# Duankaiwen/LSNet

Hardware: AMD Instinct MI355X
Metric: img/s train LSNet R-50-FPN 1333x800 bs2/GPU (higher is better)
Workload: dtype f32 (fp32-equivalent: 6 bf16 MFMA terms per product on exact 3-way operand splits, fp32 accumulate); 1 GPU; LSNet R50-FPN bbox (conv_module_type=dcn), 2 img/GPU 3x800x1344 (1333x800 padded to /32), 7 gt/img, fwd+bwd+gradient arena (the reducer's buckets, no collective on one rank)+clip35+SGD; global_batch=2, parallelism=dp1, world_size=1, memory_format=channels_last, launch=eager

## Files before the change

include/lsnet_hip.h:

```cpp
#ifndef LSNET_HIP_H_
#define LSNET_HIP_H_

#include <stdint.h>

#ifdef __cplusplus
extern "C" {
#endif

typedef struct ihipStream_t *lsn_stream_t;

typedef enum {
    LSN_OK = 0,
    LSN_ERR_INVALID = -1,
    LSN_ERR_UNSUPPORTED = -2,
    LSN_ERR_RUNTIME = -3
} lsn_status;

typedef enum { LSN_NCHW = 0, LSN_NHWC = 1 } lsn_layout;

typedef struct { int64_t b, c, h, w; } lsn_strides4;

typedef struct {
    int B, C, H, W;
    int Co, Ho, Wo;
    int kh, kw, stride, pad, dil;
    int groups, deformable_groups;
    float scale_h, scale_w;
    int mask_is_logit;
    void *workspace;
    void *gather_workspace;
    int64_t gather_workspace_bytes;
    int accumulate_param_grads;
    int out_pitch;
    int weights_prepared;
} lsn_dcn_shape;

typedef struct {
    const float *input;
    const float *offset;
    const float *mask;
    float *output;
    const float *grad_output;
    float *grad_input;
    float *grad_offset;
    float *grad_mask;
    lsn_strides4 off_st, mask_st;
    int B, H, W, Ho, Wo;
    float scale_h, scale_w;
} lsn_dcn_level;

const char *lsn_last_error(void);
int lsn_version(void);

enum { LSN_MATH_FP32 = 0, LSN_MATH_BF16X3 = 1, LSN_MATH_BF16X6 = 2, LSN_MATH_BF16 = 3 };
int lsn_set_math_mode(int mode);
int lsn_get_math_mode(void);


int lsn_dcn_forward(const lsn_dcn_shape *shape, int n_levels, const lsn_dcn_level *levels,
                    const float *weight, const float *bias, lsn_layout layout, lsn_stream_t stream);

int lsn_dcn_backward(const lsn_dcn_shape *shape, int n_levels, const lsn_dcn_level *levels,
                     const float *weight, float *grad_weight, float *grad_bias, lsn_layout layout,
                     lsn_stream_t stream);

int64_t lsn_dcn_backward_workspace_bytes(const lsn_dcn_shape *shape, int n_levels, const lsn_dcn_level *levels);
int lsn_dcn_pitched_ok(const lsn_dcn_shape *shape, int n_levels, const lsn_dcn_level *levels, int backward);
int lsn_dcn_prepared_ok(const lsn_dcn_shape *shape, int n_levels, const lsn_dcn_level *levels, int backward);
int lsn_dcn_anchor_lists(const lsn_dcn_shape *shape, int n_levels, const lsn_dcn_level *levels, lsn_layout layout,
                         int *sample_anchor, int *list_start, int *list_sample, int64_t *counts, lsn_stream_t stream);


int lsn_deform_conv_forward(const float *input, const float *weight, const float *offset, float *output,
                            int B, int C, int H, int W, int Co, int kW, int kH, int dW, int dH, int padW,
                            int padH, int dilW, int dilH, int group, int deformable_group,
                            int im2col_step, lsn_stream_t stream);
int lsn_deform_conv_backward_input(const float *input, const float *offset, const float *grad_output,
                                   float *grad_input, float *grad_offset, const float *weight, int B,
                                   int C, int H, int W, int Co, int kW, int kH, int dW, int dH, int padW,
                                   int padH, int dilW, int dilH, int group, int deformable_group,
                                   int im2col_step, lsn_stream_t stream);
int lsn_deform_conv_backward_parameters(const float *input, const float *offset, const float *grad_output,
                                        float *grad_weight, int B, int C, int H, int W, int Co, int kW,
                                        int kH, int dW, int dH, int padW, int padH, int dilW, int dilH,
                                        int group, int deformable_group, float scale, int im2col_step,
                                        lsn_stream_t stream);
int lsn_modulated_deform_conv_forward(const float *input, const float *weight, const float *bias,
                                      const float *offset, const float *mask, float *output, int B, int C,
                                      int H, int W, int Co, int kernel_h, int kernel_w, int stride_h,
                                      int stride_w, int pad_h, int pad_w, int dilation_h, int dilation_w,
                                      int group, int deformable_group, int with_bias, lsn_stream_t stream);
int lsn_modulated_deform_conv_backward(const float *input, const float *weight, const float *bias,
                                       const float *offset, const float *mask, float *grad_input,
                                       float *grad_weight, float *grad_bias, float *grad_offset,
                                       float *grad_mask, const float *grad_output, int B, int C, int H,
                                       int W, int Co, int kernel_h, int kernel_w, int stride_h,
                                       int stride_w, int pad_h, int pad_w, int dilation_h, int dilation_w,
                                       int group, int deformable_group, int with_bias,
                                       lsn_stream_t stream);
int lsn_pyramid_deform_conv_forward(const float *input, const float *weight, const float *offset,
                                    float *output, int B, int C, int H, int W, int Co, int Ho, int Wo,
                                    int kW, int kH, int dW, int dH, int padW, int padH, int dilW, int dilH,
                                    float scaleW, float scaleH, int group, int deformable_group,
                                    int im2col_step, lsn_stream_t stream);
int lsn_pyramid_deform_conv_backward_input(const float *input, const float *offset,
                                           const float *grad_output, float *grad_input,
                                           float *grad_offset, const float *weight, int B, int C, int H,
                                           int W, int Co, int Ho, int Wo, int kW, int kH, int dW, int dH,
                                           int padW, int padH, int dilW, int dilH, float scaleW,
                                           float scaleH, int group, int deformable_group,
                                           int im2col_step, lsn_stream_t stream);
int lsn_pyramid_deform_conv_backward_parameters(const float *input, const float *offset,
                                                const float *grad_output, float *grad_weight, int B,
                                                int C, int H, int W, int Co, int Ho, int Wo, int kW,
                                                int kH, int dW, int dH, int padW, int padH, int dilW,
                                                int dilH, float scaleW, float scaleH, int group,
                                                int deformable_group, float scale, int im2col_step,
                                                lsn_stream_t stream);

int lsn_sigmoid_focal_loss_forward(const float *logits, const int64_t *targets, float *losses, int N,
                                   int C, float gamma, float alpha, lsn_stream_t stream);
int lsn_sigmoid_focal_loss_backward(const float *logits, const int64_t *targets, const float *d_losses,
                                    float *d_logits, int N, int C, float gamma, float alpha,
                                    lsn_stream_t stream);
int lsn_sigmoid_focal_loss_sum(const float *logits, const int64_t *targets, const float *weight,
                               float *loss_sum, int N, int C, float gamma, float alpha,
                               lsn_stream_t stream);
int lsn_sigmoid_focal_loss_backward_weighted(const float *logits, const int64_t *targets,
                                             const float *weight, const float *scale, float *d_logits,
                                             int N, int C, float gamma, float alpha, lsn_stream_t stream);

int lsn_sigmoid_focal_loss_level_sums(const float *logits, const int64_t *targets, const float *weight, float *loss_sums,
                                      int B, int N_all, int C, int L, const int *level_starts, float gamma, float alpha,
                                      lsn_stream_t stream);
int lsn_sigmoid_focal_loss_backward_levels(const float *logits, const int64_t *targets, const float *weight, const float *scales,
                                           float *d_logits, int B, int N_all, int C, int L, const int *level_starts,
                                           float gamma, float alpha, lsn_stream_t stream);
int lsn_level_sums(const float *rows, float *sums, int B, int N_all, int L, const int *level_starts, lsn_stream_t stream);
int lsn_level_expand(const float *g, float *out_rows, int B, int N_all, int L, const int *level_starts, lsn_stream_t stream);

typedef struct {
    float *param, *grad, *momentum_buf;
    int64_t numel, first_chunk;
    int group;
} lsn_sgd_tensor;
typedef struct {
    float lr, momentum, weight_decay;
} lsn_sgd_group;
int64_t lsn_clip_sgd_workspace_bytes(void);
int lsn_clip_sgd_step(int n_tensors, const lsn_sgd_tensor *tensors_dev, int64_t total_chunks, int n_groups,
                      const lsn_sgd_group *groups, float max_norm, void *workspace, float *stats, lsn_stream_t stream);

typedef struct {
// ... 286 lines not shown
```

lsnet_amd/_lib.py:

```python
import ctypes
import os

_HERE = os.path.dirname(os.path.abspath(__file__))
SO_PATH = os.environ.get('LSNET_HIP_SO') or os.path.join(_HERE, 'csrc', 'liblsnet_hip.so')


class Strides4(ctypes.Structure):
    c_name = 'lsn_strides4'
    _fields_ = [('b', ctypes.c_int64), ('c', ctypes.c_int64), ('h', ctypes.c_int64), ('w', ctypes.c_int64)]


class DcnShape(ctypes.Structure):
    c_name = 'lsn_dcn_shape'
    _fields_ = [('B', ctypes.c_int), ('C', ctypes.c_int), ('H', ctypes.c_int), ('W', ctypes.c_int),
                ('Co', ctypes.c_int), ('Ho', ctypes.c_int), ('Wo', ctypes.c_int),
                ('kh', ctypes.c_int), ('kw', ctypes.c_int), ('stride', ctypes.c_int), ('pad', ctypes.c_int),
                ('dil', ctypes.c_int), ('groups', ctypes.c_int), ('deformable_groups', ctypes.c_int),
                ('scale_h', ctypes.c_float), ('scale_w', ctypes.c_float), ('mask_is_logit', ctypes.c_int),
                ('workspace', ctypes.c_void_p), ('gather_workspace', ctypes.c_void_p),
                ('gather_workspace_bytes', ctypes.c_int64), ('accumulate_param_grads', ctypes.c_int),
                ('out_pitch', ctypes.c_int), ('weights_prepared', ctypes.c_int)]


class DcnLevel(ctypes.Structure):
    c_name = 'lsn_dcn_level'
    _fields_ = [('input', ctypes.c_void_p), ('offset', ctypes.c_void_p), ('mask', ctypes.c_void_p),
                ('output', ctypes.c_void_p), ('grad_output', ctypes.c_void_p), ('grad_input', ctypes.c_void_p),
                ('grad_offset', ctypes.c_void_p), ('grad_mask', ctypes.c_void_p),
                ('off_st', Strides4), ('mask_st', Strides4),
                ('B', ctypes.c_int), ('H', ctypes.c_int), ('W', ctypes.c_int), ('Ho', ctypes.c_int),
                ('Wo', ctypes.c_int), ('scale_h', ctypes.c_float), ('scale_w', ctypes.c_float)]


class OffsetChainLevel(ctypes.Structure):
    c_name = 'lsn_offset_chain_level'
    _fields_ = [('off', ctypes.c_void_p), ('out', ctypes.c_void_p * 3), ('gout', ctypes.c_void_p * 6), ('goff', ctypes.c_void_p),
                ('images', ctypes.c_int64), ('per_image', ctypes.c_int64), ('off_image_pitch', ctypes.c_int64),
                ('mh', ctypes.c_float * 3), ('mw', ctypes.c_float * 3)]


class WgradBnJob(ctypes.Structure):
    c_name = 'lsn_wgrad_bn_job'
    _fields_ = [('x', ctypes.c_void_p), ('g', ctypes.c_void_p), ('w', ctypes.c_void_p), ('bn_gamma', ctypes.c_void_p),
                ('bn_mean', ctypes.c_void_p), ('bn_var', ctypes.c_void_p), ('bn_eps', ctypes.c_float),
                ('grad_w', ctypes.c_void_p), ('grad_gamma', ctypes.c_void_p), ('grad_beta', ctypes.c_void_p)]


class SgdTensor(ctypes.Structure):
    c_name = 'lsn_sgd_tensor'
    _fields_ = [('param', ctypes.c_void_p), ('grad', ctypes.c_void_p), ('momentum_buf', ctypes.c_void_p),
                ('numel', ctypes.c_int64), ('first_chunk', ctypes.c_int64), ('group', ctypes.c_int)]


class SgdGroup(ctypes.Structure):
    c_name = 'lsn_sgd_group'
    _fields_ = [('lr', ctypes.c_float), ('momentum', ctypes.c_float), ('weight_decay', ctypes.c_float)]


class ConvLevel(ctypes.Structure):
    c_name = 'lsn_conv_level'
    _fields_ = [('x', ctypes.c_void_p), ('out', ctypes.c_void_p), ('grad_out', ctypes.c_void_p),
                ('B', ctypes.c_int), ('H', ctypes.c_int), ('W', ctypes.c_int), ('residual', ctypes.c_void_p),
                ('gate', ctypes.c_void_p)]


class ConvWprep(ctypes.Structure):
    c_name = 'lsn_conv_wprep'
    _fields_ = [('kind', ctypes.c_int), ('w', ctypes.c_void_p), ('prepared', ctypes.c_void_p), ('C', ctypes.c_int),
                ('Co', ctypes.c_int), ('kh', ctypes.c_int), ('kw', ctypes.c_int), ('stride', ctypes.c_int),
                ('pad', ctypes.c_int), ('dil', ctypes.c_int),
                ('bn_gamma', ctypes.c_void_p), ('bn_var', ctypes.c_void_p), ('bn_beta', ctypes.c_void_p),
                ('bn_mean', ctypes.c_void_p), ('shift_out', ctypes.c_void_p), ('bn_eps', ctypes.c_float)]


class GnLevel(ctypes.Structure):
    c_name = 'lsn_gn_level'
    _fields_ = [('x', ctypes.c_void_p), ('y', ctypes.c_void_p), ('dy', ctypes.c_void_p), ('dx', ctypes.c_void_p),
                ('B', ctypes.c_int), ('HW', ctypes.c_int), ('y_batch_stride', ctypes.c_longlong),
                ('dy_batch_stride', ctypes.c_longlong)]


class GateJob(ctypes.Structure):
    c_name = 'lsn_gate_job'
    _fields_ = [('grad_y', ctypes.c_void_p), ('y', ctypes.c_void_p), ('grad', ctypes.c_void_p), ('B', ctypes.c_int),
                ('per_image', ctypes.c_int64), ('gy_batch_stride', ctypes.c_int64)]


class DecodeLevel(ctypes.Structure):
    c_name = 'lsn_decode_level'
    _fields_ = [('H', ctypes.c_int), ('W', ctypes.c_int), ('stride', ctypes.c_float),
                ('cls', ctypes.c_void_p), ('box', ctypes.c_void_p), ('vec', ctypes.c_void_p),
                ('cls_strides', ctypes.c_int64 * 4), ('box_strides', ctypes.c_int64 * 4), ('vec_strides', ctypes.c_int64 * 4)]


class DecodeSource(ctypes.Structure):
    c_name = 'lsn_decode_source'
    _fields_ = [('H', ctypes.c_int), ('W', ctypes.c_int), ('stride', ctypes.c_float),
                ('heat', ctypes.c_void_p), ('offset', ctypes.c_void_p),
                ('heat_strides', ctypes.c_int64 * 4), ('offset_strides', ctypes.c_int64 * 4)]


class CornerLevel(ctypes.Structure):
    c_name = 'lsn_corner_level'
    _fields_ = [('H', ctypes.c_int), ('W', ctypes.c_int), ('score', ctypes.c_void_p), ('offset', ctypes.c_void_p),
                ('score_strides', ctypes.c_int64 * 4), ('offset_strides', ctypes.c_int64 * 4),
                ('grad_score', ctypes.c_void_p), ('grad_offset', ctypes.c_void_p),
                ('grad_score_strides', ctypes.c_int64 * 4), ('grad_offset_strides', ctypes.c_int64 * 4)]


class SemLevel(ctypes.Structure):
    c_name = 'lsn_sem_level'
    _fields_ = [('H', ctypes.c_int), ('W', ctypes.c_int), ('logits', ctypes.c_void_p), ('strides', ctypes.c_int64 * 4),
                ('grad', ctypes.c_void_p), ('grad_strides', ctypes.c_int64 * 4)]


class ProfEntry(ctypes.Structure):
    c_name = 'lsn_prof_entry'
    _fields_ = [('name', ctypes.c_char * 48), ('launches', ctypes.c_longlong), ('total_ms', ctypes.c_double),
                ('flops', ctypes.c_double), ('bytes', ctypes.c_double)]


class ProfLaunch(ctypes.Structure):
    c_name = 'lsn_prof_launch'
    _fields_ = [(k, ctypes.c_int) for k in ('kind', 'C', 'Co', 'kh', 'kw', 'stride', 'pad', 'dil', 'relu', 'xpitch', 'n_levels',
                                            'has_residual', 'has_gate')] + \
               [('B', ctypes.c_int * 16), ('H', ctypes.c_int * 16), ('W', ctypes.c_int * 16), ('ms', ctypes.c_float)]


STRUCTS = (Strides4, DcnShape, DcnLevel, OffsetChainLevel, WgradBnJob, SgdTensor, SgdGroup, ConvLevel, ConvWprep, GnLevel, GateJob,
           DecodeLevel, DecodeSource, CornerLevel, SemLevel, ProfEntry, ProfLaunch)


def _signatures():
    i, q, f, d, p, c_char_p, P = ctypes.c_int, ctypes.c_int64, ctypes.c_float, ctypes.c_double, ctypes.c_void_p, \
        ctypes.c_char_p, ctypes.POINTER
    return {
        'lsn_last_error': (c_char_p, []),
        'lsn_version': (i, []),
        'lsn_set_math_mode': (i, [i]),
        'lsn_get_math_mode': (i, []),
        'lsn_dcn_forward': (i, [P(DcnShape), i, P(DcnLevel), p, p, i, p]),
        'lsn_dcn_backward': (i, [P(DcnShape), i, P(DcnLevel), p, p, p, i, p]),
        'lsn_dcn_backward_workspace_bytes': (q, [P(DcnShape), i, P(DcnLevel)]),
        'lsn_dcn_pitched_ok': (i, [P(DcnShape), i, P(DcnLevel), i]),
        'lsn_dcn_prepared_ok': (i, [P(DcnShape), i, P(DcnLevel), i]),
        'lsn_dcn_anchor_lists': (i, [P(DcnShape), i, P(DcnLevel), i, p, p, p, p, p]),
        'lsn_deform_conv_forward': (i, [p] * 4 + [i] * 16 + [p]),
        'lsn_deform_conv_backward_input': (i, [p] * 6 + [i] * 16 + [p]),
        'lsn_deform_conv_backward_parameters': (i, [p] * 4 + [i] * 15 + [f, i, p]),
        'lsn_modulated_deform_conv_forward': (i, [p] * 6 + [i] * 16 + [p]),
        'lsn_modulated_deform_conv_backward': (i, [p] * 11 + [i] * 16 + [p]),
        'lsn_pyramid_deform_conv_forward': (i, [p] * 4 + [i] * 15 + [f, f, i, i, i, p]),
        'lsn_pyramid_deform_conv_backward_input': (i, [p] * 6 + [i] * 15 + [f, f, i, i, i, p]),
        'lsn_pyramid_deform_conv_backward_parameters': (i, [p] * 4 + [i] * 15 + [f, f, i, i, f, i, p]),
        'lsn_sigmoid_focal_loss_forward': (i, [p, p, p, i, i, f, f, p]),
        'lsn_sigmoid_focal_loss_backward': (i, [p] * 4 + [i, i, f, f, p]),
        'lsn_sigmoid_focal_loss_sum': (i, [p] * 4 + [i, i, f, f, p]),
        'lsn_sigmoid_focal_loss_backward_weighted': (i, [p] * 5 + [i, i, f, f, p]),
        'lsn_sigmoid_focal_loss_level_sums': (i, [p] * 4 + [i] * 4 + [p, f, f, p]),
        'lsn_sigmoid_focal_loss_backward_levels': (i, [p] * 5 + [i] * 4 + [p, f, f, p]),
        'lsn_level_sums': (i, [p, p, i, i, i, p, p]),
        'lsn_level_expand': (i, [p, p, i, i, i, p, p]),
        'lsn_clip_sgd_workspace_bytes': (q, []),
        'lsn_clip_sgd_step': (i, [i, p, q, i, P(SgdGroup), f, p, p, p]),
        'lsn_offset_chain_forward': (i, [i, P(OffsetChainLevel), i, p]),
        'lsn_offset_chain_backward': (i, [i, P(OffsetChainLevel), i, p]),
        'lsn_topk_columns': (i, [p] + [i] * 4 + [p, p, i, i, p, p, p]),
        'lsn_assign_workspace_bytes': (q, [i] * 4),
        'lsn_centroid_assign': (i, [p, i, p, p, i, f, i] + [p] * 5),
        'lsn_centroid_assign_batch': (i, [p, i, p, p, i, p, f, i] + [p] * 5),
        'lsn_atss_assign': (i, [p, i, i, i, p, p, i, i] + [p] * 6),
        'lsn_atss_assign_batch': (i, [p, i, i, i, p, p, i, p, i] + [p] * 6),
        'lsn_dense_targets': (i, [p, i, p, i, p, p]),
        'lsn_nms_workspace_bytes': (q, [i]),
        'lsn_nms': (i, [p, p, i, f] + [p] * 4),
        'lsn_conv2d_prepared_bytes': (q, [i] * 8),
        'lsn_conv2d_prepare_weights': (i, [i, p, p] + [i] * 7 + [p]),
        'lsn_conv2d_prepare_weights_multi': (i, [i, P(ConvWprep), p]),
        'lsn_conv2d_prepare_weights_item': (i, [P(ConvWprep), p]),
        'lsn_conv2d_forward_prepared': (i, [i, P(ConvLevel), p, p] + [i] * 9 + [p]),
        'lsn_conv2d_backward_data_prepared': (i, [i, P(ConvLevel), p] + [i] * 7 + [p]),
        'lsn_conv2d_forward': (i, [p] * 5 + [i] * 11 + [p]),
        'lsn_conv2d_forward_multi': (i, [i, P(ConvLevel), p, p, p] + [i] * 8 + [p]),
        'lsn_conv2d_backward_data_multi': (i, [i, P(ConvLevel), p, p] + [i] * 7 + [p]),
        'lsn_conv2d_backward_weight_multi': (i, [i, P(ConvLevel), p, p] + [i] * 8 + [p]),
        'lsn_conv2d_forward_pitched': (i, [p] * 5 + [i] * 12 + [p]),
        'lsn_conv2d_backward_data': (i, [p] * 4 + [i] * 10 + [p]),
        'lsn_conv2d_backward_weight': (i, [p] * 4 + [i] * 11 + [p]),
        'lsn_conv2d_backward_weight_bn': (i, [p] * 6 + [f, p, p, p] + [i] * 11 + [p]),
        'lsn_conv2d_backward_weight_bn_jobs': (i, [i, P(WgradBnJob)] + [i] * 11 + [p]),
        'lsn_grouped_conv2d_forward': (i, [p] * 4 + [i] * 12 + [p]),
        'lsn_grouped_conv2d_backward_data': (i, [p, p, p] + [i] * 11 + [p]),
        'lsn_grouped_conv2d_backward_weight': (i, [p] * 4 + [i] * 12 + [p]),
        'lsn_group_norm_workspace_bytes': (q, [i, P(GnLevel), i, i]),
        'lsn_group_norm_forward': (i, [i, P(GnLevel), i, i, p, p, f, i, p, p, p]),
        'lsn_group_norm_backward': (i, [i, P(GnLevel), i, i, p, p, i] + [p] * 4 + [i, p]),
        'lsn_bn_eval_act_forward': (i, [p] * 7 + [f, i, i, i, p]),
        'lsn_bn_eval_act_workspace_bytes': (q, [i, i]),
        'lsn_bn_eval_act_backward': (i, [p] * 6 + [f, i] + [p] * 5 + [i, i, i, p]),
        'lsn_relu_gate': (i, [p, p, p, q, p]),
        'lsn_relu_gate_multi': (i, [i, P(GateJob), p]),
        'lsn_debug_phase_clocks': (i, [p, i]),
        'lsn_prof_enable': (i, [i]),
        'lsn_prof_read': (i, [P(ProfEntry), i]),
        'lsn_prof_launch_log': (i, [i]),
        'lsn_prof_read_launches': (i, [P(ProfLaunch), i]),
        'lsn_scratch_stats': (i, [p]),
        'lsn_wgrad_defer': (i, [i, p]),
        'lsn_wgrad_flush': (i, [p]),
        'lsn_selftest_mfma': (i, [p, p, p] + [i] * 4 + [p]),
        'lsn_image_prep_u8': (i, [p] + [i] * 7 + [p, p, i, f, p, i, i, p]),
        'lsn_cross_iou_bbox_forward': (i, [p] * 6 + [q, f, f, p, p]),
        'lsn_cross_iou_bbox_backward': (i, [p] * 7 + [q, f, f, p, p]),
        'lsn_cross_iou_bbox_stage_forward': (i, [p] * 5 + [q, f, f, f, p, p]),
        'lsn_cross_iou_bbox_stage_backward': (i, [p] * 6 + [q, f, f, f, p, p]),
        'lsn_cross_iou_rows_forward': (i, [i] + [p] * 7 + [q, i, i, f, f, p, p]),
        'lsn_cross_iou_rows_backward': (i, [i] + [p] * 8 + [q, i, i, f, f, p, p]),
        'lsn_cross_iou_stage_forward': (i, [i] + [p] * 6 + [q, i, i, f, f, f, p, p]),
        'lsn_cross_iou_stage_backward': (i, [i] + [p] * 7 + [q, i, i, f, f, f, p, p]),
        'lsn_pool_output_size': (i, [i] * 5),
        'lsn_max_pool2d_forward': (i, [p, i, p, i, p] + [i] * 8 + [p]),
        'lsn_max_pool2d_backward': (i, [p, i, p, p] + [i] * 9 + [p]),
        'lsn_avg_pool2d_forward': (i, [p, i, p] + [i] * 11 + [p]),
        'lsn_avg_pool2d_backward': (i, [p, i, p] + [i] * 11 + [p]),
        'lsn_upsample_add_forward': (i, [p, i, p, i, p] + [i] * 7 + [p]),
        'lsn_upsample_add_backward': (i, [p, i, p] + [i] * 8 + [p]),
        'lsn_corner_pool_forward': (i, [i, p, i, p] + [i] * 6 + [p]),
        'lsn_corner_pool_backward': (i, [i, p, i, p, i, p] + [i] * 6 + [p]),
        'lsn_decode_workspace_bytes': (q, [i, i, P(DecodeLevel), i, i]),
# ... 119 lines not shown
```

lsnet_amd/csrc/build.py:

```python
import os
import shutil
import subprocess
import sys

HERE = os.path.dirname(os.path.abspath(__file__))
SO = os.path.join(HERE, 'liblsnet_hip.so')
SOURCES = ['lib_state.hip', 'dcn.hip', 'misc.hip', 'norm.hip', 'conv.hip', 'gconv.hip', 'image.hip', 'loss.hip', 'assign.hip', 'pool.hip', 'decode.hip', 'cpv.hip']
HEADERS = ['common.h', 'lib_state.h', 'per_stream.h', 'conv_wgrad_route.h', 'conv_route.h', 'dcn_kernels.h', 'dcn_gather_kernels.h', 'dcn_sort_plan.h', 'dcn_grouped_kernels.h', 'conv_kernels.h', 'conv_wgrad_kernels.h', 'dcn_mm_kernels.h', 'prof.h', 'cross_iou_row.h', 'assign_rows.h', 'pool_rows.h', 'decode_rows.h', 'cpv_rows.h', os.path.join('..', '..', 'include', 'lsnet_hip.h')]
FLAGS = ['--offload-arch=gfx950', '-O3', '-std=c++17', '-fPIC', '-shared', '-ffp-contract=fast',
         '-fno-slp-vectorize', '-Wno-unused-result']


def kernel_signature():
    import hashlib
    h = hashlib.sha256()
    for f in ('common.h', 'conv_kernels.h', 'conv_wgrad_kernels.h', 'conv_wgrad_route.h', 'conv_route.h', 'conv.hip', 'dcn_kernels.h', 'dcn_gather_kernels.h', 'dcn_sort_plan.h', 'dcn_mm_kernels.h', 'dcn_grouped_kernels.h', 'dcn.hip'):
        with open(os.path.join(HERE, f), 'rb') as fh:
            h.update(fh.read())
    return h.hexdigest()[:16]


def _hipcc():
    for c in (shutil.which('hipcc'), '/opt/rocm/bin/hipcc'):
        if c and os.path.exists(c):
            return c
    raise RuntimeError('hipcc not found: liblsnet_hip.so cannot be built')


OBJ_DIR = os.path.join(HERE, 'build')
UNIT_HEADERS = {
    'lib_state.hip': ['common.h', 'lib_state.h', 'per_stream.h', 'conv_wgrad_route.h', 'prof.h'],
    'dcn.hip': ['common.h', 'lib_state.h', 'per_stream.h', 'conv_wgrad_route.h', 'conv_route.h', 'dcn_kernels.h', 'dcn_gather_kernels.h', 'dcn_sort_plan.h', 'dcn_mm_kernels.h', 'dcn_grouped_kernels.h', 'conv_kernels.h', 'prof.h'],
    'conv.hip': ['common.h', 'lib_state.h', 'per_stream.h', 'conv_wgrad_route.h', 'conv_route.h', 'conv_kernels.h', 'conv_wgrad_kernels.h', 'prof.h'],
    'misc.hip': ['common.h', 'lib_state.h', 'per_stream.h', 'conv_wgrad_route.h', 'prof.h'], 'norm.hip': ['common.h', 'lib_state.h', 'per_stream.h', 'conv_wgrad_route.h', 'prof.h'],
    'gconv.hip': ['common.h', 'prof.h'],
    'image.hip': ['common.h'], 'loss.hip': ['common.h', 'cross_iou_row.h'], 'assign.hip': ['common.h', 'assign_rows.h'],
    'pool.hip': ['common.h', 'pool_rows.h'], 'decode.hip': ['common.h', 'decode_rows.h', 'pool_rows.h', 'prof.h'], 'cpv.hip': ['common.h', 'assign_rows.h', 'cpv_rows.h'],
}
UNIT_FLAGS = {'assign.hip': ['-ffp-contract=off'], 'decode.hip': ['-ffp-contract=off'], 'cpv.hip': ['-ffp-contract=off']}
API_HEADER = os.path.join('..', '..', 'include', 'lsnet_hip.h')


def _stale(target, deps):
    if not os.path.exists(target):
        return True
    t = os.path.getmtime(target)
    return any(os.path.exists(d) and os.path.getmtime(d) > t for d in deps)


def _unit_deps(src):
    return [os.path.join(HERE, f) for f in [src] + UNIT_HEADERS.get(src, HEADERS) + [API_HEADER]] + [os.path.abspath(__file__)]


def needs_build(so=None, obj_dir=None):
    so = so or SO
    obj_dir = obj_dir or OBJ_DIR
    if not os.path.exists(so):
        return True
    return any(_stale(os.path.join(obj_dir, s + '.o'), _unit_deps(s)) for s in SOURCES) or \
        _stale(so, [os.path.join(obj_dir, s + '.o') for s in SOURCES])


def build(force=False, verbose=False, defines=(), so=None):
    so = so or SO
    obj_dir = OBJ_DIR if so == SO else so + '.build'
    if not force and not needs_build(so, obj_dir):
        return so
    os.makedirs(obj_dir, exist_ok=True)
    cc = _hipcc()
    cflags = [f for f in FLAGS if f != '-shared'] + ['-D' + d for d in defines]
    jobs = []
    for s in SOURCES:
        obj = os.path.join(obj_dir, s + '.o')
        if force or _stale(obj, _unit_deps(s)):
            cmd = [cc] + cflags + UNIT_FLAGS.get(s, []) + ['-c', os.path.join(HERE, s), '-o', obj]
            if verbose:
                print(' '.join(cmd), file=sys.stderr)
            jobs.append((s, subprocess.Popen(cmd, cwd=HERE)))
    failed = [s for s, p in jobs if p.wait() != 0]
    if failed:
        raise RuntimeError('hipcc failed for ' + ', '.join(failed))
    cmd = [cc, '--offload-arch=gfx950', '-shared', '-fPIC'] + [os.path.join(obj_dir, s + '.o') for s in SOURCES] + ['-o', so]
    if verbose:
        print(' '.join(cmd), file=sys.stderr)
    subprocess.check_call(cmd, cwd=HERE)
    return so


HOST_SO = os.path.join(HERE, 'liblsnet_host.so')
HOST_SOURCES = [os.path.join('host', 'rle.cpp'), os.path.join('host', 'coco_match.cpp'),
                os.path.join('host', 'image.cpp'), os.path.join('host', 'nms_host.cpp')]
HOST_HEADERS = [os.path.join('..', '..', 'include', 'lsnet_host.h')]


def build_host(force=False, verbose=False):
    deps = [os.path.join(HERE, f) for f in HOST_SOURCES + HOST_HEADERS]
    if not force and os.path.exists(HOST_SO) and all(os.path.getmtime(d) <= os.path.getmtime(HOST_SO) for d in deps):
        return HOST_SO
    cxx = shutil.which('g++') or shutil.which('c++')
    if cxx is None:
        raise RuntimeError('g++ not found: liblsnet_host.so cannot be built')
    cmd = [cxx, '-O3', '-std=c++17', '-fPIC', '-shared', '-Wall', '-ffp-contract=off'] + \
        [os.path.join(HERE, s) for s in HOST_SOURCES] + ['-o', HOST_SO]
    if verbose:
        print(' '.join(cmd), file=sys.stderr)
    subprocess.check_call(cmd, cwd=HERE)
    return HOST_SO


if __name__ == '__main__':
    print(build(force='--force' in sys.argv, verbose=True))
    print(build_host(force='--force' in sys.argv, verbose=True))
```

lsnet_amd/csrc/dcn.hip:

```cpp
#include <limits.h>
#include <string.h>

#include <vector>

#include "conv_route.h"
#include "dcn_kernels.h"
#include "dcn_mm_kernels.h"
#include "dcn_grouped_kernels.h"
#include "lib_state.h"
#include "prof.h"

namespace lsn {

static long long *g_dbg_buf = nullptr;
static int g_dbg_block = 0;
static bool dbg_on(int bit) { return (g_dbg_block & bit) != 0; }

static double dcn_flops(const DcnArgs &a)
{
    double px = 0;
    for (int i = 0; i < a.nlv; ++i) px += (double)a.lv[i].B * a.lv[i].Ho * a.lv[i].Wo;
    return 2.0 * px * a.Co * (a.C / a.groups) * a.kh * a.kw;
}

// ... 428 lines not shown
            constexpr int long_thr = 40;
            is_long[j] = !all_anchor || gsamp[j] > (int64_t)long_thr * nanch;
        }
        for (int pass = 0; pass < 2; ++pass) {
            for (int j = 0; j < ga.ng; ++j) {
                const GatherGrp &G = ga.g[j];
                if (!to_anchor[j] || is_long[j] != (pass == 0)) continue;
                AnchorGrp &A = aa.g[aa.ng++];
                A.gx = G.gx, A.x = G.x, A.B = G.B, A.H = G.H, A.W = G.W, A.abase = G.abase, A.a0 = aa.NA;
                aa.NA += G.B * (G.H + 1) * (G.W + 1);
                pl.anchor_pixels += G.B * G.H * G.W;
            }
            if (pass == 0) pl.na_long = aa.NA;
        }
        for (int j = 0; j < ga.ng; ++j) {
            if (to_anchor[j]) continue;
            const GatherGrp &G = ga.g[j];
            keep[nk] = G;
            keep[nk].blk0 = (int)q;
            q += (int64_t)G.B * cdiv(G.H, GT) * cdiv(G.W, GT);
            pl.block_samples += gsamp[j];
            ++nk;
        }
        for (int j = 0; j < nk; ++j) ga.g[j] = keep[j];
        ga.ng = nk;
        Q = q;
    }
    ga.NB = (int)Q;
    ga.C = a.C, ga.K = K, ga.KD = KD, ga.dg = a.dg;
    aa.C = a.C, aa.K = K, aa.KD = KD, aa.dg = a.dg;
    size_t o = 0;
    pl.o_gcol = o, o = align256(o + (size_t)prow * K * a.C * sizeof(float));
    pl.o_hist = o, o = align256(o + ds_hist_ints(pl.nsamples, pl.nanchors) * sizeof(int));
    pl.o_start = o, o = align256(o + ((size_t)pl.nanchors + 1) * sizeof(int));
    pl.o_key = o, o = align256(o + (size_t)pl.nsamples * sizeof(int));
    pl.o_ent = o, o = align256(o + (size_t)pl.nsamples * sizeof(GEntry));
    pl.o_gtap = o, o = align256(o + ((size_t)pl.nsamples + 1) * sizeof(Tap));
    pl.o_S = o, o = align256(o + (size_t)pl.aa.NA * 4 * a.C * sizeof(float));
    const int ncb_max = (ga.NB == 0 && aa.ng > 0 && a.C > 256) ? cdiv(a.C, 256) : 1;
    aa.ncb = dbg_on(LSN_DBG_ANCHOR_ONE_WAVE) ? 1 : ncb_max;
    aa.hb_slot = (long long)pl.nsamples * 4;
    pl.o_H = o, o = align256(o + (size_t)pl.nsamples * 4 * sizeof(float) * ncb_max);
    pl.o_pairs = o, o = align256(o + (size_t)pl.nsamples * 2 * sizeof(int2));
    pl.bytes = o;
    pl.ok = true;
}

static int wgrad_splits(int cols, int per_cu)
{
    const int slots = 256 * per_cu;
    int s = slots / cols;
    return s < 1 ? 1 : s;
}

static bool mm_wgrad_ok(const DcnArgs &a) { return mm_common_ok(a) && a.Co % 256 == 0 && (a.C / a.dg) % 64 == 0; }
static bool wgrad_mm_image_ok(const DcnArgs &a, int nchunks) { return fits_i32((int64_t)nchunks * 2 * (a.Co / 32) * mm_npl(), 1024); }

static bool grouped_wgrad_ok(const DcnArgs &a)
{
    if (a.groups <= 1 || a.C % a.groups != 0 || a.Co != a.C || a.kh * a.kw > 9) return false;
    const int cg = a.C / a.groups;
    if (!(cg == 4 || cg == 8 || cg == 16 || cg == 32) || ((int64_t)a.C * cg) % 256 != 0 || a.C % a.dg != 0) return false;
    const int nch = cg >= 16 ? cg : 256 / cg;
    if ((a.C / a.dg) % nch != 0 || a.C % nch != 0) return false;
    return grouped_inputs_ok(a);
}

enum FwdKernel { FWD_MM, FWD_GROUPED, FWD_XN_PLANES, FWD_XN, FWD_FP32 };
enum DataKernel { DATA_NONE, GATHER_GROUPED, GATHER_MM, GATHER_XN, SCATTER_XN, SCATTER_FP32 };
enum WgradKernel { WG_NONE, WG_GROUPED, WG_MM, WG_XN_ORDERED, WG_XN_ATOMIC, WG_FP32_ORDERED, WG_FP32_ATOMIC };
enum WeightImage { IMG_NONE, IMG_FRAGMENT, IMG_PLANES, IMG_PLANES_T };

struct DcnRoute {
    FwdKernel fwd = FWD_FP32;
    DataKernel data = DATA_NONE;
    WgradKernel wgrad = WG_NONE;
    WeightImage image = IMG_NONE;
    bool pitched = false;
    bool prepared = false;
    int gcol_ks = 0;
    int wg_steps = 0;
    bool own_gather_ws = false;
    GatherPlan plan;
    bool gather() const { return data == GATHER_GROUPED || data == GATHER_MM || data == GATHER_XN; }
};

static DcnRoute route_forward(const DcnArgs &a, const lsn_dcn_shape &s, lsn_layout layout)
{
    DcnRoute r;
    const int np = math_np();
    if (s.workspace && mm_fwd_ok(a)) {
        r.fwd = FWD_MM, r.image = IMG_FRAGMENT;
    } else if (grouped_fwd_ok(a)) {
        r.fwd = FWD_GROUPED;
    } else if (np != 0 && xn_ok(a) && xn_lds_bytes(split_npl(np), a.kh * a.kw * a.dg) <= 160 * 1024) {
        r.fwd = FWD_XN;
        if (s.workspace && (a.C / a.groups) % 8 == 0) r.fwd = FWD_XN_PLANES, r.image = IMG_PLANES;
    }
    r.pitched = r.prepared = layout == LSN_NHWC && r.fwd == FWD_MM;
    return r;
}

static int gcol_mfma_ksteps(const DcnArgs &a)
{
    const int Cg = a.C / a.groups, Cog = a.Co / a.groups;
    if (a.C % GC_COLS != 0 || a.opitch % 4 != 0) return 0;
    for (int i = 0; i < a.nlv; ++i)
        if ((reinterpret_cast<uintptr_t>(a.lv[i].gout) & 15) != 0) return 0;
    if (a.groups == 1) return (a.Co == 64 || a.Co == 128 || a.Co == 256) ? a.Co / 4 : 0;
    return (Cog == Cg && (Cg == 4 || Cg == 8 || Cg == 16 || Cg == 32)) ? (Cg == 32 ? 8 : 4) : 0;
}

static int wgrad_split_grid(const DcnArgs &a, int nsteps, int *ncol, int *nz)
{
    const int K = a.kh * a.kw, Cg = a.C / a.groups, Cog = a.Co / a.groups;
    *ncol = a.groups * K * (Cg / a.SL) * cdiv(a.SL, WG_BN), *nz = cdiv(Cog, WG_BM);
    int s = wgrad_splits(*ncol * *nz, 2);
    if (s > nsteps) s = nsteps;
    if (s < 1) s = 1;
    return s > 65535 ? 65535 : s;
}

static DcnRoute route_backward(DcnArgs &a, const lsn_dcn_shape &s, lsn_layout layout, const void *gws, size_t gws_bytes,
                               bool want_wgrad)
{
    DcnRoute r;
    const int np = math_np(), K = a.kh * a.kw;
    bool any_data = false;
    for (int i = 0; i < a.nlv; ++i) any_data = any_data || a.lv[i].gx || a.lv[i].goff || a.lv[i].gmsk;
    if (any_data) {
        const bool can_split = s.workspace && np && a.groups == 1 && a.Co % 2 == 0;
        const bool grouped = bwd_grouped_ok(a), mm = mm_bwd_ok(a), x3 = can_split && bwd_x3_ok(a);
        const DataKernel cand = !bwd_colbuf_env()                         ? DATA_NONE
                                : grouped                                 ? GATHER_GROUPED
                                : (can_split && mm && bwd_offsets_ok(a)) ? GATHER_MM
                                : x3                                      ? GATHER_XN
                                                                          : DATA_NONE;
        bool fits = false;
        if (cand != DATA_NONE && (gws || layout == LSN_NCHW)) {
            gather_plan(a, r.plan, mm || grouped);
            r.own_gather_ws = !gws && r.plan.ok;
            fits = r.plan.ok && (r.own_gather_ws || r.plan.bytes <= gws_bytes);
        }
        r.data = fits ? cand : x3 ? SCATTER_XN : SCATTER_FP32;
        if (r.data == GATHER_GROUPED) r.gcol_ks = gcol_mfma_ksteps(a);
        r.image = r.data == GATHER_MM ? IMG_FRAGMENT : can_split ? IMG_PLANES_T : IMG_NONE;
        r.prepared = layout == LSN_NHWC && r.data == GATHER_MM;
    }
    if (want_wgrad) {
        int64_t rows = 0, steps = 0;
        for (int i = 0; i < a.nlv; ++i) rows += a.lv[i].P, steps += cdiv(a.lv[i].P, WG_BP);
        r.wg_steps = (int)steps;
        const size_t nW = (size_t)a.Co * K * (a.C / a.groups);
        const bool tap_table = r.gather() && (r.own_gather_ws || ((reinterpret_cast<uintptr_t>(gws) + r.plan.o_gtap) & 15) == 0);
        if (grouped_wgrad_ok(a) && a.opitch == a.Co && nW % 4 == 0 && rows < ((int64_t)1 << 30)) {
            r.wgrad = WG_GROUPED;
        } else if (mm_wgrad_ok(a) && tap_table && wgrad_mm_image_ok(a, r.wg_steps)) {
            r.wgrad = WG_MM;
        } else {
            int ncol, nz;
            const int splits = wgrad_split_grid(a, r.wg_steps, &ncol, &nz);
            const bool ordered = nW % 4 == 0 && (size_t)splits * (nW + a.Co) * sizeof(float) <= ((size_t)256 << 20);
            r.wgrad = np ? (ordered ? WG_XN_ORDERED : WG_XN_ATOMIC) : (ordered ? WG_FP32_ORDERED : WG_FP32_ATOMIC);
        }
    }
    r.pitched = layout == LSN_NHWC && r.data == GATHER_MM && (!want_wgrad || r.wgrad == WG_MM);
    return r;
}

static int bwd_tap_groups(const DcnArgs &a)
{
    const int K = a.kh * a.kw;
    int best = 1;
    double best_cost = 1e30;
    for (int g = 1; g <= K; ++g) {
        if (K % g) continue;
        const double cost = (double)cdiv(a.ntiles * g, 512) / g * (1.0 + 0.05 * g);
        if (cost < best_cost - 1e-9) best_cost = cost, best = g;
    }
    return best;
}

struct SideStream {
    hipStream_t side = nullptr;
    hipEvent_t fork = nullptr, join = nullptr;
};
static PerStream<SideStream> g_side;
static int side_stream(hipStream_t st, SideStream **out)
{
    return g_side.get(st, "side streams", out, [&](SideStream &S) {
        if (int rc = refuse_capture(st, "side stream would be created")) return rc;
        int lo = 0, hi = 0;
        LSN_HIP(hipDeviceGetStreamPriorityRange(&lo, &hi));
        LSN_HIP(hipStreamCreateWithPriority(&S.side, hipStreamNonBlocking, hi));
        LSN_HIP(hipEventCreateWithFlags(&S.fork, hipEventDisableTiming));
        LSN_HIP(hipEventCreateWithFlags(&S.join, hipEventDisableTiming));
        return 0;
    });
}

static int build_lists(DcnArgs &a, const GatherPlan &pl, unsigned char *ws, hipStream_t st)
{
    int *hist = reinterpret_cast<int *>(ws + pl.o_hist), *start = reinterpret_cast<int *>(ws + pl.o_start);
    int *key = reinterpret_cast<int *>(ws + pl.o_key);
    int2 *pairs[2] = {reinterpret_cast<int2 *>(ws + pl.o_pairs), reinterpret_cast<int2 *>(ws + pl.o_pairs) + pl.nsamples};
    GEntry *ent = reinterpret_cast<GEntry *>(ws + pl.o_ent);
    Tap *gtap = reinterpret_cast<Tap *>(ws + pl.o_gtap);
    const int KD = a.kh * a.kw * a.dg, n = pl.nsamples, na = pl.nanchors;
    a.gtap_rows = n / KD;
    const int db = ds_digit_bits(na), passes = ds_passes(na), nblocks = ds_blocks(n);
    const dim3 grid(nblocks), block(DS_THREADS), kblock(DS_KEY_THREADS);
    const size_t lds = ds_scatter_lds_bytes(db);
    hipLaunchKernelGGL(dcn_list_keys_kernel, grid, kblock, 0, st, a, n, na, db, nblocks, key, hist, gtap);
    a.gtap = gtap;
    for (int p = 0; p < passes; ++p) {
        const int2 *in = p > 0 ? pairs[(p - 1) & 1] : nullptr;
        int2 *out = pairs[p & 1];
        if (p > 0) hipLaunchKernelGGL(dcn_list_hist_kernel, grid, kblock, 0, st, n, p, db, nblocks, in, hist);
        hipLaunchKernelGGL(dcn_list_scan_kernel, dim3(1 << db), block, 0, st, hist, db, nblocks);
        if (p == 0)
            hipLaunchKernelGGL((dcn_list_scatter_kernel<true, false>), grid, block, lds, st, n, na, p, db, nblocks, hist, key, in, out,
                               ent, (int *)nullptr, gtap, KD, a.gtap_rows);
        else if (p + 1 < passes)
            hipLaunchKernelGGL((dcn_list_scatter_kernel<false, false>), grid, block, lds, st, n, na, p, db, nblocks, hist, key, in, out,
                               ent, (int *)nullptr, gtap, KD, a.gtap_rows);
        else
            hipLaunchKernelGGL((dcn_list_scatter_kernel<false, true>), grid, block, lds, st, n, na, p, db, nblocks, hist, key, in,
                               (int2 *)nullptr, ent, reinterpret_cast<int *>(out), gtap, KD, a.gtap_rows);
    }
    const int *skey = reinterpret_cast<const int *>(pairs[(passes - 1) & 1]);
    hipLaunchKernelGGL(dcn_list_starts_kernel, dim3(cdiv(na + 1, 256)), dim3(256), 0, st, n, na, skey, start);
    LSN_HIP(hipGetLastError());
    return 0;
}

static int launch_bwd_gather(DcnArgs &a, DcnRoute &r, unsigned char *ws, hipStream_t st_main)
{
    GatherPlan &pl = r.plan;
    a.gcol = reinterpret_cast<float *>(ws + pl.o_gcol);
    int *start = reinterpret_cast<int *>(ws + pl.o_start);
    GEntry *ent = reinterpret_cast<GEntry *>(ws + pl.o_ent);
    SideStream *side = nullptr;
    if (r.data == GATHER_MM)
        if (int rc = side_stream(st_main, &side)) return rc;
    hipStream_t st = side ? side->side : st_main;
    if (side) {
        LSN_HIP(hipEventRecord(side->fork, st_main));
        LSN_HIP(hipStreamWaitEvent(side->side, side->fork, 0));
    }
    if (int rc = build_lists(a, pl, ws, st)) return rc;
    if (side) {
        LSN_HIP(hipEventRecord(side->join, side->side));
        st = st_main;
    }
    bool any_off = false;
    for (int i = 0; i < a.nlv; ++i) any_off = any_off || a.lv[i].goff || a.lv[i].gmsk;
    float *Hb = nullptr;
    switch (r.data) {
    case GATHER_GROUPED:
        if (r.gcol_ks) {
            DcnArgs g = a;
            const int nred = a.groups == 1 ? a.Co : GC_COLS;
            const size_t lds = dcn_gcol_mfma_lds_bytes(nred);
            const dim3 grid(number_tiles(g, GC_PX) * (a.C / GC_COLS));
            int rc = 0;
            switch (r.gcol_ks) {
            case 4: rc = launch256(dcn_gcol_mfma_kernel<4>, grid, lds, st, g, nred); break;
            case 8: rc = launch256(dcn_gcol_mfma_kernel<8>, grid, lds, st, g, nred); break;
            case 16: rc = launch256(dcn_gcol_mfma_kernel<16>, grid, lds, st, g, nred); break;
            case 32: rc = launch256(dcn_gcol_mfma_kernel<32>, grid, lds, st, g, nred); break;
            default: rc = launch256(dcn_gcol_mfma_kernel<64>, grid, lds, st, g, nred); break;
            }
            if (rc) return rc;
        } else {
            const long long nquads = (long long)pl.nsamples / a.dg * (a.C / 4);
            const int blocks = (int)((nquads + 255) / 256 < 16384 ? (nquads + 255) / 256 : 16384);
            hipLaunchKernelGGL(dcn_gcol_grouped_kernel, dim3(blocks > 0 ? blocks : 1), dim3(256), 0, st, a, nquads);
        }
        if (any_off) Hb = reinterpret_cast<float *>(ws + pl.o_H);
        break;
    case GATHER_MM: {
        const float *xs[MAXLV];
        float *outs[MAXLV];
        int rows[MAXLV];
        for (int i = 0; i < a.nlv; ++i) {
            xs[i] = a.lv[i].gout;
            outs[i] = a.gcol + (size_t)a.lv[i].prow0 * a.kh * a.kw * a.C;
            rows[i] = a.lv[i].P;
        }
        if (int rc = conv_mm_rows(a.nlv, xs, outs, rows, a.Co, a.opitch, a.kh * a.kw * a.C, a.wtp, st)) return rc;
        LSN_HIP(hipStreamWaitEvent(st_main, side->join, 0));
        if (any_off) Hb = reinterpret_cast<float *>(ws + pl.o_H);
        break;
    }
    default:
        if (int rc = split_dispatch(math_np(), [&](auto npc) {
                constexpr int NP = decltype(npc)::value;
                return launch256(dcn_bwd_data_xn_kernel<NP, true>, dim3(a.ntiles, bwd_tap_groups(a)), bwd_xn_lds_bytes(NP, a.kh * a.kw * a.dg), st, a);
            }))
            return rc;
        break;
    }
    pl.ga.raw = pl.aa.raw = r.data != GATHER_XN ? 1 : 0;
    pl.ga.Hb = pl.aa.Hb = Hb;
    pl.ga.gcol = a.gcol, pl.ga.start = start, pl.ga.ent = ent;
    if (pl.aa.ng > 0) {
        pl.aa.gcol = a.gcol, pl.aa.start = start, pl.aa.ent = ent;
        pl.aa.S = reinterpret_cast<float *>(ws + pl.o_S);
        if (pl.na_long > 0)
            hipLaunchKernelGGL(dcn_anchor_sum_kernel<4>, dim3(pl.na_long, pl.aa.ncb), dim3(256), 0, st, pl.aa, 0, pl.na_long);
        if (pl.aa.NA > pl.na_long)
            hipLaunchKernelGGL(dcn_anchor_sum_kernel<1>, dim3(cdiv(pl.aa.NA - pl.na_long, 4), pl.aa.ncb), dim3(256), 0, st, pl.aa,
                               pl.na_long, pl.aa.NA - pl.na_long);
        hipLaunchKernelGGL(dcn_anchor_combine_kernel, dim3(cdiv(pl.anchor_pixels, 4)), dim3(256), 0, st, pl.aa, pl.anchor_pixels);
    }
    if (pl.ga.NB > 0) {
        const bool split = pl.block_samples > (int64_t)300 * pl.ga.NB;
        if (split)
            hipLaunchKernelGGL(dcn_gather_kernel<4>, dim3(pl.ga.NB), dim3(256), 0, st, pl.ga);
        else
            hipLaunchKernelGGL(dcn_gather_kernel<1>, dim3(cdiv(pl.ga.NB, 4)), dim3(256), 0, st, pl.ga);
    }
    if (Hb)
        hipLaunchKernelGGL(dcn_offgrad_kernel, dim3(cdiv(pl.nsamples, 256)), dim3(256), 0, st, a, pl.nsamples,
                           reinterpret_cast<const float4 *>(Hb), pl.aa.ng > 0 ? pl.aa.ncb : 1);
    LSN_HIP(hipGetLastError());
    return 0;
}

static int launch_bwd_data(DcnArgs &a, DcnRoute &r, void *gather_ws, hipStream_t st)
{
    ProfScope prof(PROF_BWD_DATA, a, st);
    if (r.gather()) return launch_bwd_gather(a, r, reinterpret_cast<unsigned char *>(gather_ws), st);
    for (int i = 0; i < a.nlv; ++i)
        if (a.lv[i].gx)
            LSN_HIP(hipMemsetAsync(a.lv[i].gx, 0, sizeof(float) * (size_t)a.lv[i].B * a.lv[i].H * a.lv[i].W * a.C, st));
    if (r.data == SCATTER_XN)
        return split_dispatch(math_np(), [&](auto npc) {
            constexpr int NP = decltype(npc)::value;
            return launch256(dcn_bwd_data_xn_kernel<NP, false>, dim3(a.ntiles, bwd_tap_groups(a)), bwd_xn_lds_bytes(NP, a.kh * a.kw * a.dg), st, a);
        });
    return (a.Co / a.groups > 64) ? launch_bwd_data_t<256>(a, st) : launch_bwd_data_t<64>(a, st);
}

static int wgrad_vec_bits(const DcnArgs &a)
{
    bool vx = a.C % 2 == 0, vg = a.Co % 2 == 0;
    for (int i = 0; i < a.nlv; ++i) {
        const Lvl &L = a.lv[i];
        vx = vx && (reinterpret_cast<uintptr_t>(L.x) & 7) == 0 && (long long)L.B * L.H * L.W * a.C < (1ll << 29);
        vg = vg && (reinterpret_cast<uintptr_t>(L.gout) & 7) == 0 && (long long)(L.P + WG_BP) * a.Co < (1ll << 29);
    }
    return (vx ? 1 : 0) | (vg ? 2 : 0);
}

static int launch_wgrad_mm(const DcnArgs &a_in, int nchunks, bool accumulate, hipStream_t st, const ConvWgradCall *dense = nullptr)
{
    DcnArgs a = a_in;
    const int K = a.kh * a.kw, npl = mm_npl();
    const size_t nW = (size_t)a.Co * K * a.C;
    const size_t img_bytes = (size_t)nchunks * 2 * (a.Co / 32) * npl * 1024;
    const int ncol = K * (a.C / 64), nz = a.Co / 256;
    int S = (512 + ncol * nz / 2) / (ncol * nz);
    if (S > nchunks / 4) S = nchunks / 4;
    if (S < 1) S = 1;
    const int nsteps16 = 2 * nchunks;
    int spb = cdiv(nsteps16, 256);
    if (spb < 4) spb = 4;
    const int nblk_s = cdiv(nsteps16, spb);
    const size_t img_f = (img_bytes + 15) / 16 * 4, part_f = (size_t)S * nW, pb_f = ((size_t)nblk_s * a.Co + 3) & ~(size_t)3;
    const size_t meta_f = ((size_t)nchunks * 8 + 64 + 3) & ~(size_t)3;
    size_t tap_entries = 0;
    if (dense) {
        a.gtap_rows = number_rows(a);
// ... 180 lines not shown
            a.lv[i].out = out_tmp[i];
        }
    }
    a.bias = bias;
    const DcnRoute r = route_forward(a, s, layout);
    if (a.opitch != a.Co && !r.pitched)
        return fail(LSN_ERR_UNSUPPORTED, "deformable forward: out_pitch %d != Co %d outside the matrix-pipe kernels "
                    "(lsn_dcn_pitched_ok)", a.opitch, a.Co);
    if (s.weights_prepared && !r.prepared)
        return fail(LSN_ERR_UNSUPPORTED, "deformable forward: weights_prepared outside the matrix-pipe kernels (lsn_dcn_prepared_ok)");
    if (int rc = prepare_image(a, r.image, s, false, st)) return rc;
    int rc = 0;
    switch (r.fwd) {
    case FWD_MM: rc = launch_forward_mm(a, st); break;
    case FWD_GROUPED: rc = launch_forward_grouped(a, st); break;
    case FWD_XN_PLANES: rc = launch_forward_xn(a, true, st); break;
    case FWD_XN: rc = launch_forward_xn(a, false, st); break;
    case FWD_FP32: rc = launch_forward_fp32(a, st); break;
    }
    if (rc) return rc;
    if (layout == LSN_NCHW)
        for (int i = 0; i < n; ++i)
            if (int rc = permute_rs(out_tmp[i], lv[i].output, lv[i].B, lv[i].Ho * lv[i].Wo, s.Co, st)) return rc;
    return 0;
}

static int dcn_backward_impl(const lsn_dcn_shape &s, int n, const lsn_dcn_level *lv, const float *weight,
                             float *grad_weight, float *grad_bias, lsn_layout layout, hipStream_t st)
{
    if (int rc = check_shape(s)) return rc;
    LSN_CHECK(weight != nullptr, "weight is NULL");
    if (grad_bias && !grad_weight)
        return fail(LSN_ERR_UNSUPPORTED, "grad_bias without grad_weight is not supported");
    DcnArgs a;
    if (int rc = fill_levels(a, s, n, lv, BWD_BM)) return rc;
    Scratch ws(st);
    const int K = s.kh * s.kw, Cg = s.C / s.groups;
    std::vector<float *> gx_tmp(n, nullptr);
    float *gw_tmp = nullptr;
    for (int i = 0; i < n; ++i) LSN_CHECK(lv[i].input && lv[i].grad_output, "level %d: input/grad_output is NULL", i);
    if (layout == LSN_NHWC) {
        a.w = weight;
        a.gw = grad_weight;
        for (int i = 0; i < n; ++i) {
            a.lv[i].x = lv[i].input;
            a.lv[i].gout = lv[i].grad_output;
            a.lv[i].gx = lv[i].grad_input;
        }
    } else {
        float *w2 = ws.get((size_t)s.Co * Cg * K);
        if (!w2) return fail(LSN_ERR_RUNTIME, "workspace allocation failed");
        if (int rc = permute_rs(weight, w2, s.Co, Cg, K, st)) return rc;
        a.w = w2;
        if (grad_weight) {
            gw_tmp = ws.get((size_t)s.Co * Cg * K);
            if (!gw_tmp) return fail(LSN_ERR_RUNTIME, "workspace allocation failed");
            a.gw = gw_tmp;
        }
        for (int i = 0; i < n; ++i) {
            float *x2 = ws.get(n_in(s, lv[i])), *g2 = ws.get(n_out(s, lv[i]));
            if (!x2 || !g2) return fail(LSN_ERR_RUNTIME, "workspace allocation failed");
            if (int rc = permute_rs(lv[i].input, x2, lv[i].B, s.C, lv[i].H * lv[i].W, st)) return rc;
            if (int rc = permute_rs(lv[i].grad_output, g2, lv[i].B, s.Co, lv[i].Ho * lv[i].Wo, st)) return rc;
            a.lv[i].x = x2;
            a.lv[i].gout = g2;
            if (lv[i].grad_input) {
                gx_tmp[i] = ws.get(n_in(s, lv[i]));
                if (!gx_tmp[i]) return fail(LSN_ERR_RUNTIME, "workspace allocation failed");
                a.lv[i].gx = gx_tmp[i];
            }
        }
    }
    a.gb = grad_bias;

    void *gws = s.gather_workspace;
    DcnRoute r = route_backward(a, s, layout, gws, gather_ws_bytes(s), a.gw != nullptr);
    if (a.opitch != a.Co && r.data == DATA_NONE)
        return fail(LSN_ERR_UNSUPPORTED, "deformable backward: out_pitch without a data-gradient pass");
    if (a.opitch != a.Co && !r.pitched)
        return fail(LSN_ERR_UNSUPPORTED, "deformable backward: out_pitch %d != Co %d outside the matrix-pipe kernels "
                    "(lsn_dcn_pitched_ok)", a.opitch, a.Co);
    if (s.weights_prepared && r.data != DATA_NONE && !r.prepared)
        return fail(LSN_ERR_UNSUPPORTED, "deformable backward: weights_prepared outside the matrix-pipe kernels (lsn_dcn_prepared_ok)");
    if (r.data != DATA_NONE) {
        if (r.own_gather_ws && !(gws = ws.get(r.plan.bytes / 4 + 64)))
            return fail(LSN_ERR_RUNTIME, "workspace allocation failed");
        if (int rc = prepare_image(a, r.image, s, true, st)) return rc;
        if (int rc = launch_bwd_data(a, r, gws, st)) return rc;
    }
    if (r.wgrad != WG_NONE)
        if (int rc = launch_wgrad(a, r, s.accumulate_param_grads != 0 && layout == LSN_NHWC, st)) return rc;
    if (layout == LSN_NCHW) {
        for (int i = 0; i < n; ++i)
            if (gx_tmp[i])
                if (int rc = permute_rs(gx_tmp[i], lv[i].grad_input, lv[i].B, lv[i].H * lv[i].W, s.C, st)) return rc;
        if (gw_tmp)
            if (int rc = permute_rs(gw_tmp, grad_weight, s.Co, K, Cg, st)) return rc;
    }
    return 0;
}

static lsn_strides4 nchw_strides(int Ch, int H, int W)
{
    lsn_strides4 s;
    s.b = (int64_t)Ch * H * W;
    s.c = (int64_t)H * W;
    s.h = W;
    s.w = 1;
    return s;
}

static int make_single(lsn_dcn_shape &s, lsn_dcn_level &L, int B, int C, int H, int W, int Co, int Ho, int Wo,
                       int kH, int kW, int dH, int dW, int padH, int padW, int dilH, int dilW, int group, int dg,
                       float scaleH, float scaleW, bool pyramid)
{
    if (dH != dW || padH != padW || dilH != dilW)
        return fail(LSN_ERR_UNSUPPORTED, "different stride/pad/dilation for h and w is not supported");
    memset(&s, 0, sizeof(s));
    memset(&L, 0, sizeof(L));
    LSN_CHECK(kH > 0 && kW > 0, "kernel size should be greater than zero, but got kH: %d kW: %d", kH, kW);
    LSN_CHECK(dH > 0, "stride should be greater than zero, but got dH: %d dW: %d", dH, dW);
    LSN_CHECK(dilH > 0, "dilation should be greater than 0, but got dilationH: %d dilationW: %d", dilH, dilW);
    if (!pyramid) {
        Ho = conv_out(H, kH, dH, padH, dilH);
        Wo = conv_out(W, kW, dW, padW, dilW);
    } else {
        LSN_CHECK(conv_out(Ho, kH, dH, padH, dilH) == Ho && conv_out(Wo, kW, dW, padW, dilW) == Wo,
                  "invalid spatial size of offset, expected height: %d width: %d, but got height: %d width: %d",
                  conv_out(Ho, kH, dH, padH, dilH), conv_out(Wo, kW, dW, padW, dilW), Ho, Wo);
    }
    LSN_CHECK(Ho >= 1 && Wo >= 1,
              "Given input size: (%d x %d x %d). Calculated output size: (%d x %d x %d). Output size is too small",
              C, H, W, Co, Ho, Wo);
    LSN_CHECK(H >= kH && W >= kW, "input image is smaller than kernel");
    s.B = B; s.C = C; s.H = H; s.W = W; s.Co = Co; s.Ho = Ho; s.Wo = Wo;
    s.kh = kH; s.kw = kW; s.stride = dH; s.pad = padH; s.dil = dilH;
    s.groups = group; s.deformable_groups = dg;
    s.scale_h = scaleH; s.scale_w = scaleW;
    L.B = B; L.H = H; L.W = W; L.Ho = Ho; L.Wo = Wo;
    L.scale_h = scaleH; L.scale_w = scaleW;
    L.off_st = nchw_strides(dg * 2 * kH * kW, Ho, Wo);
    L.mask_st = nchw_strides(dg * kH * kW, Ho, Wo);
    return 0;
}

static_assert(CW_MAXLV <= MAXLV && CW_STEP_PX == WG_BP, "conv_wgrad_route.h counts the k-steps of these kernels");
bool general_gemms_only() { return !dcn_mm_env(); }

static int conv_dcn_args(DcnArgs &a, const ConvWgradCall &c)
{
    const ConvWgradShape &s = c.s;
    a = DcnArgs{};
    int steps = 0;
    for (int i = 0; i < s.n; ++i) {
        Lvl &L = a.lv[i];
        L.x = c.x[i], L.gout = c.go[i];
        L.B = s.lv[i].B, L.H = s.lv[i].H, L.W = s.lv[i].W, L.Ho = s.lv[i].Ho, L.Wo = s.lv[i].Wo, L.P = s.lv[i].P, L.sh = L.sw = 1.f;
        L.tile0 = steps;
        steps += cdiv(L.P, WG_BP);
    }
    a.nlv = s.n;
    a.C = s.C, a.Co = s.Co, a.kh = s.kh, a.kw = s.kw, a.stride = s.stride, a.pad = c.pad, a.dil = s.dil, a.groups = 1, a.dg = 1;
    a.SL = s.C;
    a.opitch = s.Co;
    a.gw = c.gw, a.gb = c.gb;
    return steps;
// ... 58 lines not shown
                          LSN_DBG_ATOMIC_SCATTER | LSN_DBG_WG_COMPUTED_TAPS | LSN_DBG_WG_SCALAR_LOADS | LSN_DBG_GENERAL_GEMMS;
    if (word & ~known) return fail(LSN_ERR_INVALID, "lsn_debug_phase_clocks: unknown debug bits 0x%x", (unsigned)(word & ~known));
    lsn::g_dbg_buf = device_buf_512;
    lsn::g_dbg_block = word;
    return 0;
}

static bool query_args(lsn::DcnArgs &a, const lsn_dcn_shape *shape, int n_levels, const lsn_dcn_level *levels, int backward)
{
    using namespace lsn;
    if (!shape || !levels || check_shape(*shape) != 0) return false;
    if (fill_levels(a, *shape, n_levels, levels, backward ? BWD_BM : 64) != 0) return false;
    for (int i = 0; i < n_levels; ++i) {
        a.lv[i].x = levels[i].input;
        a.lv[i].gout = levels[i].grad_output;
        a.lv[i].gx = levels[i].grad_input;
    }
    return true;
}

int64_t lsn_dcn_backward_workspace_bytes(const lsn_dcn_shape *shape, int n_levels, const lsn_dcn_level *levels)
{
    using namespace lsn;
    DcnArgs a;
    if (!query_args(a, shape, n_levels, levels, 1)) return 0;
    lsn_dcn_shape s = *shape;
    s.workspace = &s;
    const DcnRoute r = route_backward(a, s, LSN_NHWC, &s, SIZE_MAX, false);
    return r.gather() ? (int64_t)r.plan.bytes : 0;
}

int lsn_dcn_prepared_ok(const lsn_dcn_shape *shape, int n_levels, const lsn_dcn_level *levels, int backward)
{
    using namespace lsn;
    DcnArgs a;
    if (!query_args(a, shape, n_levels, levels, backward)) return 0;
    if (!backward) return route_forward(a, *shape, LSN_NHWC).prepared ? 1 : 0;
    return route_backward(a, *shape, LSN_NHWC, shape->gather_workspace, gather_ws_bytes(*shape), false).prepared ? 1 : 0;
}

int lsn_dcn_pitched_ok(const lsn_dcn_shape *shape, int n_levels, const lsn_dcn_level *levels, int backward)
{
    using namespace lsn;
    DcnArgs a;
    if (!query_args(a, shape, n_levels, levels, backward)) return 0;
    if (!backward) return route_forward(a, *shape, LSN_NHWC).pitched ? 1 : 0;
    return route_backward(a, *shape, LSN_NHWC, shape->gather_workspace, gather_ws_bytes(*shape), true).pitched ? 1 : 0;
}

int lsn_dcn_anchor_lists(const lsn_dcn_shape *shape, int n_levels, const lsn_dcn_level *levels, lsn_layout layout,
                         int *sample_anchor, int *list_start, int *list_sample, int64_t *counts, lsn_stream_t stream)
{
    using namespace lsn;
    if (!shape || !levels || !counts) return fail(LSN_ERR_INVALID, "shape/levels/counts is NULL");
    const lsn_dcn_shape &s = *shape;
    hipStream_t st = reinterpret_cast<hipStream_t>(stream);
    if (int rc = check_shape(s)) return rc;
    DcnArgs a;
    if (layout != LSN_NHWC) return fail(LSN_ERR_UNSUPPORTED, "lsn_dcn_anchor_lists: LSN_NHWC only");
    if (int rc = fill_levels(a, s, n_levels, levels, BWD_BM)) return rc;
    for (int i = 0; i < n_levels; ++i) {
        LSN_CHECK(levels[i].input && levels[i].grad_output, "level %d: input/grad_output is NULL", i);
        a.lv[i].x = levels[i].input;
        a.lv[i].gout = levels[i].grad_output;
        a.lv[i].gx = levels[i].grad_input;
    }
    void *gws = s.gather_workspace;
    DcnRoute r = route_backward(a, s, layout, gws, gather_ws_bytes(s), false);
    if (!r.gather()) return fail(LSN_ERR_UNSUPPORTED, "lsn_dcn_anchor_lists: this call builds no anchor lists (route without the gather pass)");
    const GatherPlan &pl = r.plan;
    counts[0] = pl.nsamples, counts[1] = pl.nanchors;
    if (!sample_anchor && !list_start && !list_sample) return 0;
    LSN_CHECK(sample_anchor && list_start && list_sample, "lsn_dcn_anchor_lists: all three outputs or none");
    unsigned char *w = reinterpret_cast<unsigned char *>(gws);
    if (int rc = build_lists(a, pl, w, st)) return rc;
    const int n = pl.nsamples > pl.nanchors + 1 ? pl.nsamples : pl.nanchors + 1;
    hipLaunchKernelGGL(dcn_list_export_kernel, dim3(cdiv(n, 256)), dim3(256), 0, st, pl.nsamples, pl.nanchors,
                       reinterpret_cast<const int *>(w + pl.o_key), reinterpret_cast<const int *>(w + pl.o_start),
                       reinterpret_cast<const GEntry *>(w + pl.o_ent), sample_anchor, list_start, list_sample);
    LSN_HIP(hipGetLastError());
    return 0;
}

int lsn_dcn_forward(const lsn_dcn_shape *shape, int n_levels, const lsn_dcn_level *levels, const float *weight,
                    const float *bias, lsn_layout layout, lsn_stream_t stream)
{
    if (!shape || !levels) return fail(LSN_ERR_INVALID, "shape/levels is NULL");
    return dcn_forward_impl(*shape, n_levels, levels, weight, bias, layout, stream);
}

int lsn_dcn_backward(const lsn_dcn_shape *shape, int n_levels, const lsn_dcn_level *levels, const float *weight,
                     float *grad_weight, float *grad_bias, lsn_layout layout, lsn_stream_t stream)
{
    if (!shape || !levels) return fail(LSN_ERR_INVALID, "shape/levels is NULL");
    return dcn_backward_impl(*shape, n_levels, levels, weight, grad_weight, grad_bias, layout, stream);
}

int lsn_deform_conv_forward(const float *input, const float *weight, const float *offset, float *output, int B,
                            int C, int H, int W, int Co, int kW, int kH, int dW, int dH, int padW, int padH,
                            int dilW, int dilH, int group, int deformable_group, int im2col_step,
                            lsn_stream_t stream)
{
    (void)im2col_step;
    lsn_dcn_shape s;
    lsn_dcn_level L;
    if (int rc = make_single(s, L, B, C, H, W, Co, 0, 0, kH, kW, dH, dW, padH, padW, dilH, dilW, group,
                             deformable_group, 1.f, 1.f, false))
        return rc;
    L.input = input; L.offset = offset; L.output = output;
    return dcn_forward_impl(s, 1, &L, weight, nullptr, LSN_NCHW, stream);
}

int lsn_deform_conv_backward_input(const float *input, const float *offset, const float *grad_output,
                                   float *grad_input, float *grad_offset, const float *weight, int B, int C,
                                   int H, int W, int Co, int kW, int kH, int dW, int dH, int padW, int padH,
                                   int dilW, int dilH, int group, int deformable_group, int im2col_step,
                                   lsn_stream_t stream)
{
    (void)im2col_step;
    lsn_dcn_shape s;
    lsn_dcn_level L;
    if (int rc = make_single(s, L, B, C, H, W, Co, 0, 0, kH, kW, dH, dW, padH, padW, dilH, dilW, group,
                             deformable_group, 1.f, 1.f, false))
        return rc;
    L.input = input; L.offset = offset; L.grad_output = grad_output;
    L.grad_input = grad_input; L.grad_offset = grad_offset;
    return dcn_backward_impl(s, 1, &L, weight, nullptr, nullptr, LSN_NCHW, stream);
}

static int scale_weight_grad(float *gw, size_t n, float scale, hipStream_t st)
{
    if (scale == 1.f) return 0;
    hipLaunchKernelGGL(scale_kernel, dim3(256), dim3(256), 0, st, gw, n, scale);
    LSN_HIP(hipGetLastError());
    return 0;
}

int lsn_deform_conv_backward_parameters(const float *input, const float *offset, const float *grad_output,
                                        float *grad_weight, int B, int C, int H, int W, int Co, int kW, int kH,
                                        int dW, int dH, int padW, int padH, int dilW, int dilH, int group,
                                        int deformable_group, float scale, int im2col_step, lsn_stream_t stream)
{
    (void)im2col_step;
    lsn_dcn_shape s;
    lsn_dcn_level L;
    if (int rc = make_single(s, L, B, C, H, W, Co, 0, 0, kH, kW, dH, dW, padH, padW, dilH, dilW, group,
                             deformable_group, 1.f, 1.f, false))
        return rc;
    L.input = input; L.offset = offset; L.grad_output = grad_output;
    if (int rc = dcn_backward_impl(s, 1, &L, grad_weight, grad_weight, nullptr, LSN_NCHW, stream)) return rc;
    return scale_weight_grad(grad_weight, (size_t)Co * (C / group) * kH * kW, scale, stream);
}

int lsn_modulated_deform_conv_forward(const float *input, const float *weight, const float *bias,
                                      const float *offset, const float *mask, float *output, int B, int C, int H,
                                      int W, int Co, int kernel_h, int kernel_w, int stride_h, int stride_w,
                                      int pad_h, int pad_w, int dilation_h, int dilation_w, int group,
                                      int deformable_group, int with_bias, lsn_stream_t stream)
{
    lsn_dcn_shape s;
    lsn_dcn_level L;
    if (int rc = make_single(s, L, B, C, H, W, Co, 0, 0, kernel_h, kernel_w, stride_h, stride_w, pad_h, pad_w,
                             dilation_h, dilation_w, group, deformable_group, 1.f, 1.f, false))
        return rc;
    LSN_CHECK(mask != nullptr, "mask is NULL");
    L.input = input; L.offset = offset; L.mask = mask; L.output = output;
// ... 76 lines not shown
```

lsnet_amd/csrc/dcn_gather_kernels.h:

```cpp
#pragma once
#include "dcn_sort_plan.h"

namespace lsn {

struct __align__(16) GEntry {
    int s;
    int pad;
    float ly, lx;
};

struct GatherGrp {
    float *gx;
    const float *x;
    int B, H, W;
    int abase;
    int blk0;
};
struct GatherArgs {
    GatherGrp g[MAXLV];
    int ng, NB;
    int C, K, KD, dg;
    const float *gcol;
    const int *start;
    const GEntry *ent;
    int raw;
    float *Hb;
};

struct AnchorGrp {
    float *gx;
    const float *x;
    int B, H, W;
    int abase;
    int a0;
};
struct AnchorArgs {
    AnchorGrp g[MAXLV];
    int ng, NA;
    int C, K, KD, dg;
    const float *gcol;
    const int *start;
    const GEntry *ent;
    float *S;
    int raw;
    float *Hb;
    int ncb;
    long long hb_slot;
};

template <int CTRL>
__device__ __forceinline__ float dpp_f32(float v)
{
    return __int_as_float(__builtin_amdgcn_update_dpp(0, __float_as_int(v), CTRL, 0xf, 0xf, true));
}
__device__ __forceinline__ float wave64_sum16(const float (&d)[16], int lane)
{
    const bool b0 = lane & 1, b1 = lane & 2, b2 = lane & 4, b3 = lane & 8;
    float w[8], w2[4], z[2];
#pragma unroll
    for (int i = 0; i < 8; ++i) w[i] = (b0 ? d[2 * i + 1] : d[2 * i]) + dpp_f32<0xB1>(b0 ? d[2 * i] : d[2 * i + 1]);
#pragma unroll
    for (int i = 0; i < 4; ++i) w2[i] = (b1 ? w[2 * i + 1] : w[2 * i]) + dpp_f32<0x4E>(b1 ? w[2 * i] : w[2 * i + 1]);
#pragma unroll
    for (int i = 0; i < 2; ++i) z[i] = (b2 ? w2[2 * i + 1] : w2[2 * i]) + dpp_f32<0x124>(b2 ? w2[2 * i] : w2[2 * i + 1]);
    float r = (b3 ? z[1] : z[0]) + dpp_f32<0x128>(b3 ? z[0] : z[1]);
    r += __shfl_xor(r, 16);
    r += __shfl_xor(r, 32);
    return r;
}

__device__ __forceinline__ const Lvl &find_level_by_row(const DcnArgs &a, int prow)
{
    int li = 0;
    while (li + 1 < a.nlv && prow >= a.lv[li + 1].prow0) ++li;
    return a.lv[li];
}

__global__ __launch_bounds__(256) void dcn_gcol_grouped_kernel(const DcnArgs a, long long nquads)
{
    const int K = a.kh * a.kw, C = a.C, Cg = C / a.groups, Cog = a.Co / a.groups, C4 = C >> 2;
    for (long long id = blockIdx.x * (long long)blockDim.x + threadIdx.x; id < nquads; id += (long long)gridDim.x * blockDim.x) {
        const long long row = id / C4;
        const int c = (int)(id - row * C4) * 4;
        const int prow = (int)(row / K), k = (int)(row - (long long)prow * K);
        const Lvl &L = find_level_by_row(a, prow);
        const int g = c / Cg, ci = c - g * Cg;
        const float *go = L.gout + (size_t)(prow - L.prow0) * a.Co + (size_t)g * Cog;
        const float *w = a.w + ((size_t)g * Cog * K + k) * Cg + ci;
        float4 s = make_float4(0.f, 0.f, 0.f, 0.f);
        for (int j = 0; j < Cog; ++j) {
            const float gv = go[j];
            const float4 wv = *reinterpret_cast<const float4 *>(w + (size_t)j * K * Cg);
            s.x = fmaf(gv, wv.x, s.x), s.y = fmaf(gv, wv.y, s.y), s.z = fmaf(gv, wv.z, s.z), s.w = fmaf(gv, wv.w, s.w);
        }
        *reinterpret_cast<float4 *>(a.gcol + (size_t)row * C + c) = s;
    }
}


__global__ __launch_bounds__(DS_KEY_THREADS) void dcn_list_keys_kernel(const DcnArgs a, int nsamples, int nanchors, int db, int nblocks,
                                                                       int *__restrict__ key, int *__restrict__ hist,
                                                                       Tap *__restrict__ gtap)
{
    constexpr int PER = DS_BLOCK / DS_KEY_THREADS;
    __shared__ int h[DS_MAX_DIGITS];
    const int ndig = 1 << db;
    for (int d = threadIdx.x; d < ndig; d += DS_KEY_THREADS) h[d] = 0;
    __syncthreads();
    const int K = a.kh * a.kw, KD = K * a.dg;
    const Lvl *lv[PER];
    TapRaw raw[PER];
    int prow[PER], kd[PER];
#pragma unroll
    for (int r = 0; r < PER; ++r) {
        const int s = blockIdx.x * DS_BLOCK + r * DS_KEY_THREADS + threadIdx.x;
        const int sc = s < nsamples ? s : nsamples - 1;
        prow[r] = sc / KD, kd[r] = sc - prow[r] * KD;
        const int dgi = kd[r] / K;
        lv[r] = &find_level_by_row(a, prow[r]);
        raw[r] = tap_raw(a, *lv[r], prow[r] - lv[r]->prow0, kd[r] - dgi * K, dgi);
    }
#pragma unroll
    for (int r = 0; r < PER; ++r) {
        const int s = blockIdx.x * DS_BLOCK + r * DS_KEY_THREADS + threadIdx.x;
        if (s >= nsamples) continue;
        const Lvl &L = *lv[r];
        const int dgi = kd[r] / K, k = kd[r] - dgi * K;
        int4 yx = make_int4(0, 0, 0, 0);
        const Tap t = tap_finish(a, L, prow[r] - L.prow0, k, raw[r], &yx);
        gtap[(size_t)kd[r] * a.gtap_rows + prow[r]] = t;
        if (s == 0) {
            Tap z = {};
            gtap[(size_t)KD * a.gtap_rows] = z;
        }
        int anchor = nanchors;
        if (L.gx != nullptr && t.flags) {
            const int y0 = (t.flags & 3) ? yx.x : -1, x0 = (t.flags & 5) ? yx.y : -1;
            const int HWo = L.Ho * L.Wo;
            const int b = (prow[r] - L.prow0) / HWo;
            anchor = L.abase + (b * (L.H + 1) + y0 + 1) * (L.W + 1) + x0 + 1;
        }
        key[s] = anchor;
        atomicAdd(&h[ds_digit(anchor, 0, db)], 1);
    }
    __syncthreads();
    for (int d = threadIdx.x; d < ndig; d += DS_KEY_THREADS) hist[ds_hist_at(d, blockIdx.x, nblocks)] = h[d];
}

__global__ __launch_bounds__(DS_KEY_THREADS) void dcn_list_hist_kernel(int nsamples, int pass, int db, int nblocks,
                                                                       const int2 *__restrict__ in, int *__restrict__ hist)
{
    constexpr int PER = DS_BLOCK / DS_KEY_THREADS;
    __shared__ int h[DS_MAX_DIGITS];
    const int ndig = 1 << db;
    for (int d = threadIdx.x; d < ndig; d += DS_KEY_THREADS) h[d] = 0;
    __syncthreads();
    int kk[PER];
#pragma unroll
    for (int r = 0; r < PER; ++r) {
        const int i = blockIdx.x * DS_BLOCK + r * DS_KEY_THREADS + threadIdx.x;
        kk[r] = i < nsamples ? in[i].x : 0;
    }
#pragma unroll
    for (int r = 0; r < PER; ++r)
        if (blockIdx.x * DS_BLOCK + r * DS_KEY_THREADS + threadIdx.x < nsamples) atomicAdd(&h[ds_digit(kk[r], pass, db)], 1);
    __syncthreads();
    for (int d = threadIdx.x; d < ndig; d += DS_KEY_THREADS) hist[ds_hist_at(d, blockIdx.x, nblocks)] = h[d];
}

__device__ __forceinline__ int block_exclusive_sum(int v, int *wsum, int *total)
{
    const int lane = threadIdx.x & 63, wave = threadIdx.x >> 6;
    int x = v;
#pragma unroll
    for (int o = 1; o < 64; o <<= 1) {
        const int y = __shfl_up(x, o);
        if (lane >= o) x += y;
    }
    if (lane == 63) wsum[wave] = x;
    __syncthreads();
    int before = 0, all = 0;
#pragma unroll
    for (int w = 0; w < DS_WAVES; ++w) {
        const int t = wsum[w];
        before += w < wave ? t : 0;
        all += t;
    }
    __syncthreads();
    *total = all;
    return before + x - v;
}

__global__ __launch_bounds__(DS_THREADS) void dcn_list_scan_kernel(int *__restrict__ hist, int db, int nblocks)
{
    __shared__ int wsum[DS_WAVES];
    int *row = hist + ds_hist_at(blockIdx.x, 0, nblocks);
    int carry = 0;
    for (int base = 0; base < nblocks; base += DS_THREADS) {
        const int i = base + threadIdx.x;
        const int v = i < nblocks ? row[i] : 0;
        int total;
        const int ex = block_exclusive_sum(v, wsum, &total);
        if (i < nblocks) row[i] = carry + ex;
        carry += total;
    }
    if (threadIdx.x == 0) hist[ds_hist_at(1 << db, 0, nblocks) + blockIdx.x] = carry;
}

template <bool FIRST, bool LAST>
__global__ __launch_bounds__(DS_THREADS) void dcn_list_scatter_kernel(int nsamples, int nanchors, int pass, int db, int nblocks,
                                                                      const int *__restrict__ hist, const int *__restrict__ key_in,
                                                                      const int2 *__restrict__ in, int2 *__restrict__ out,
                                                                      GEntry *__restrict__ ent, int *__restrict__ skey,
                                                                      const Tap *__restrict__ gtap, int KD, int gtap_rows)
{
    extern __shared__ int ds_lds[];
    __shared__ int wsum[DS_WAVES];
    const int lane = threadIdx.x & 63, wave = threadIdx.x >> 6;
    const int ndig = 1 << db, blk = blockIdx.x;
    int *const cnt = ds_lds, *const gbase = ds_lds + DS_WAVES * ndig;
    int k[DS_ROWS], v[DS_ROWS], loc[DS_ROWS];
#pragma unroll
    for (int r = 0; r < DS_ROWS; ++r) {
        const int i = ds_elem(blk, wave, r, lane);
        k[r] = 0, v[r] = 0;
        if (i < nsamples) {
            if constexpr (FIRST) {
                k[r] = key_in[i], v[r] = i;
            } else {
                const int2 p = in[i];
                k[r] = p.x, v[r] = p.y;
            }
        }
    }
    for (int d = threadIdx.x; d < DS_WAVES * ndig; d += DS_THREADS) cnt[d] = 0;
    {
        const int *tot = hist + ds_hist_at(ndig, 0, nblocks);
        const int per = ndig > DS_THREADS ? ndig / DS_THREADS : 1;
        const int d0 = threadIdx.x * per;
        int sum = 0;
        for (int j = 0; j < per; ++j) sum += d0 + j < ndig ? tot[d0 + j] : 0;
        int total;
        int run = block_exclusive_sum(sum, wsum, &total);
        for (int j = 0; j < per; ++j)
            if (d0 + j < ndig) {
                gbase[d0 + j] = run + hist[ds_hist_at(d0 + j, blk, nblocks)];
                run += tot[d0 + j];
            }
    }
    __syncthreads();
    volatile int *cw = cnt + wave * ndig;
#pragma unroll
    for (int r = 0; r < DS_ROWS; ++r) {
        const bool valid = ds_elem(blk, wave, r, lane) < nsamples;
        const int d = ds_digit(k[r], pass, db);
        unsigned long long m = __ballot(valid);
        for (int b = 0; b < db; ++b) {
            const bool bit = (d >> b) & 1;
            const unsigned long long bal = __ballot(bit);
            m &= bit ? bal : ~bal;
        }
        const int rank = __popcll(m & ((1ull << lane) - 1ull));
        const int prior = valid ? cw[d] : 0;
        loc[r] = prior + rank;
        __builtin_amdgcn_wave_barrier();
        if (valid && rank == 0) cw[d] = prior + __popcll(m);
        __builtin_amdgcn_wave_barrier();
    }
    __syncthreads();
    for (int d = threadIdx.x; d < ndig; d += DS_THREADS) {
        int before = 0;
#pragma unroll
        for (int w = 0; w < DS_WAVES; ++w) {
            const int c = cnt[w * ndig + d];
            cnt[w * ndig + d] = before;
            before += c;
        }
    }
    __syncthreads();
#pragma unroll
    for (int r = 0; r < DS_ROWS; ++r) {
        const int i = ds_elem(blk, wave, r, lane);
        if (i >= nsamples) continue;
        const int d = ds_digit(k[r], pass, db);
        const int pos = ds_position(gbase[d], cnt[wave * ndig + d], loc[r]);
        if ((unsigned)pos >= (unsigned)nsamples) continue;
        if constexpr (LAST) {
            skey[pos] = k[r];
            const int s = v[r];
            if (k[r] != nanchors && (unsigned)s < (unsigned)nsamples) {
                const int prow = s / KD, kd = s - prow * KD;
                const float4 t = reinterpret_cast<const float4 *>(gtap + ((size_t)kd * gtap_rows + prow))[1];
                GEntry e;
                e.s = s, e.pad = __float_as_int(t.z);
                e.ly = t.x, e.lx = t.y;
                ent[pos] = e;
            }
        } else {
            out[pos] = make_int2(k[r], v[r]);
        }
    }
}

__global__ void dcn_list_starts_kernel(int nsamples, int nanchors, const int *__restrict__ skey, int *__restrict__ start)
{
    const int an = blockIdx.x * blockDim.x + threadIdx.x;
    if (an > nanchors) return;
    int lo = 0, hi = nsamples;
    while (lo < hi) {
        const int mid = lo + ((hi - lo) >> 1);
        if (skey[mid] < an) lo = mid + 1;
        else hi = mid;
    }
    start[an] = lo;
}

__global__ void dcn_list_export_kernel(int nsamples, int nanchors, const int *__restrict__ key, const int *__restrict__ start,
                                       const GEntry *__restrict__ ent, int *__restrict__ sample_anchor, int *__restrict__ list_start,
                                       int *__restrict__ list_sample)
{
    const int i = blockIdx.x * blockDim.x + threadIdx.x;
    if (i < nsamples) {
        const int k = key[i];
        sample_anchor[i] = k == nanchors ? -1 : k;
        list_sample[i] = i < start[nanchors] ? ent[i].s : -1;
    }
    if (i <= nanchors) list_start[i] = start[i];
}

constexpr int GT = 4;
template <int NW>
__global__ __launch_bounds__(256) void dcn_gather_kernel(const GatherArgs ga)
{
    constexpr int GU = 4;
    __shared__ float4 accs[4][GT * GT][64];
    const int lane = threadIdx.x & 63, wave_id = threadIdx.x >> 6;
    const int wave = NW == 4 ? wave_id : 0;
    const int C = ga.C, K = ga.K, KD = ga.KD;
    const int cpdg = C / ga.dg;
    const int bi = NW == 4 ? ga.NB - 1 - xcd_remap(blockIdx.x, gridDim.x) : xcd_remap(blockIdx.x, gridDim.x) * 4 + wave_id;
    if (bi >= ga.NB) return;
    int gi = 0;
    while (gi + 1 < ga.ng && bi >= ga.g[gi + 1].blk0) ++gi;
    const GatherGrp &G = ga.g[gi];
    const int nbx = (G.W + GT - 1) / GT, nby = (G.H + GT - 1) / GT;
    const int lb_ = bi - G.blk0;
    const int b = lb_ / (nbx * nby), rem = lb_ - b * nbx * nby;
    const int y0 = (rem / nbx) * GT, x0 = (rem % nbx) * GT;
    float4(*acc)[64] = accs[wave_id];
    for (int cb = 0; cb < C; cb += 256) {
        const int c = cb + lane * 4;
#pragma unroll
        for (int p = 0; p < GT * GT; ++p) acc[p][lane] = make_float4(0.f, 0.f, 0.f, 0.f);
        int grp = 0;
        for (int an_i = 0; an_i < (GT + 1) * (GT + 1); ++an_i) {
            const int ai = an_i / (GT + 1), aj = an_i - ai * (GT + 1);
            const int ay = y0 - 1 + ai, ax = x0 - 1 + aj;
            if (ay > G.H - 1 || ax > G.W - 1) continue;
            const int an = G.abase + (b * (G.H + 1) + ay + 1) * (G.W + 1) + ax + 1;
            const int lb = __builtin_amdgcn_readfirstlane(ga.start[an]);
            const int le = __builtin_amdgcn_readfirstlane(ga.start[an + 1]);
            if (lb == le) continue;
            bool inb[2][2];
            float4 xa[2][2], S[2][2];
#pragma unroll
            for (int dy = 0; dy < 2; ++dy)
#pragma unroll
                for (int dx = 0; dx < 2; ++dx) {
                    const int pi = ai - 1 + dy, pj = aj - 1 + dx;
                    inb[dy][dx] = pi >= 0 && pi < GT && pj >= 0 && pj < GT && y0 + pi < G.H && x0 + pj < G.W;
                    S[dy][dx] = make_float4(0.f, 0.f, 0.f, 0.f);
                    xa[dy][dx] = make_float4(0.f, 0.f, 0.f, 0.f);
                    if (ga.Hb != nullptr && inb[dy][dx] && c < C)
                        xa[dy][dx] = *reinterpret_cast<const float4 *>(G.x + ((size_t)(b * G.H + ay + dy) * G.W + ax + dx) * C + c);
                }
            for (int base = lb; base < le; base += 64) {
                const int n = min(64, le - base);
                const int ngrp = (n + GU - 1) / GU;
                const int first = (wave - grp) & (NW - 1);
                grp += ngrp;
                if (first >= ngrp) continue;
                GEntry e = {};
                if (lane < n) e = ga.ent[base + lane];
                for (int j0 = first * GU; j0 < n; j0 += NW * GU) {
                    float4 v[GU];
                    float ly[GU], lx[GU], mm[GU];
#pragma unroll
                    for (int u = 0; u < GU; ++u) {
                        const int j = min(j0 + u, n - 1);
                        const int s = __builtin_amdgcn_readlane(e.s, j);
                        ly[u] = __int_as_float(__builtin_amdgcn_readlane(__float_as_int(e.ly), j));
                        lx[u] = __int_as_float(__builtin_amdgcn_readlane(__float_as_int(e.lx), j));
                        mm[u] = ga.raw ? __int_as_float(__builtin_amdgcn_readlane(e.pad, j)) : 1.f;
                        int row = s, c_lo = 0, c_hi = C;
                        if (ga.dg > 1) {
                            const int prow = s / KD, kd = s - prow * KD;
                            const int dgi = kd / K;
                            row = prow * K + (kd - dgi * K);
                            c_lo = dgi * cpdg, c_hi = c_lo + cpdg;
                        }
                        const bool on = (j0 + u < n) && c < c_hi && c >= c_lo;
                        v[u] = *reinterpret_cast<const float4 *>(ga.gcol + (size_t)row * C + (c < C ? c : 0));
                        if (!on) v[u] = make_float4(0.f, 0.f, 0.f, 0.f);
                    }
#pragma unroll
                    for (int u = 0; u < GU; ++u) {
                        const float hy = 1.f - ly[u], hx = 1.f - lx[u];
#pragma unroll
// ... 252 lines not shown
```

lsnet_amd/models/dense_heads/ls_head.py:

```python
import math
import os

import numpy as np
import torch
import torch.nn as nn

from ...cnn import ConvModule, bias_init_with_prob, kaiming_init, normal_init
from ...ops.conv import Conv2d
from ...ops.group_norm import GroupNorm
from ...core import PointGenerator, assigners, build_assigner, build_sampler, multiclass_nms_lsvr
from ...ops.backend import get_backend
from ...ops import ModulatedDeformConvPack, PyramidDeformConv
from ...ops.dcn import offset_scale_chain
from ...ops import cross_iou as fused_ciou
from ...ops.focal import level_rows_ok, level_sums
from ...ops.streams import side_stream
from ..builder import HEADS, build_loss

FUSED_LEVEL_SUMS = os.environ.get('LSNET_FUSED_LEVEL_SUMS', '1') != '0'
SIDE_STREAM_TARGETS = os.environ.get('LSNET_SIDE_STREAM_TARGETS', '1') != '0'
NATIVE_DECODE = os.environ.get('LSNET_NATIVE_DECODE', '1') != '0'
DECODE_CAND_CAP = 16384

TASK_BRANCHES = {'bbox': ('bbox',), 'segm': ('segm',), 'pose_bbox': ('bbox', 'pose'), 'pose_kbox': ('pose',)}


class DCNConvModule(nn.Module):

    def __init__(self, in_channels=256, out_channels=256, kernel_size=3, dilation=1, num_groups=1, dcn_pad=1):
        super().__init__()
        self.conv = ModulatedDeformConvPack(in_channels, out_channels, kernel_size, 1, dcn_pad)
        self.bn = GroupNorm(num_groups, out_channels)
        self.relu = nn.ReLU(inplace=True)

    def forward(self, x):
        return self.bn.forward_act(self.conv(x))

    def forward_multi(self, xs):
        return self.bn.forward_multi(self.conv.forward_multi(xs), relu=True)


def _split_px_views(x, shapes):
    B, C = x.shape[:2]
    flat = x.permute(0, 2, 3, 1).reshape(B, -1, C)
    outs, o = [], 0
    for h, w in shapes:
        outs.append(flat[:, o:o + h * w].reshape(B, h, w, C).permute(0, 3, 1, 2))
        o += h * w
    return outs


class _SplitPxFn(torch.autograd.Function):

    @staticmethod
    def forward(ctx, x, shapes):
        ctx.shapes, ctx.dims = shapes, (x.shape[0], x.shape[1])
        return tuple(_split_px_views(x, shapes))

    @staticmethod
    def backward(ctx, *grads):
        B, C = ctx.dims
        ref = next(g for g in grads if g is not None)
        parts = [g.permute(0, 2, 3, 1).reshape(B, h * w, C) if g is not None else ref.new_zeros((B, h * w, C))
                 for g, (h, w) in zip(grads, ctx.shapes)]
        flat = torch.cat(parts, dim=1)
        return flat.unsqueeze(2).permute(0, 3, 1, 2), None


class LevelTerms(list):

    def __init__(self, base):
        super().__init__(base.unbind(0))
        self.base = base


def _signed_pairs(t, dim):
    neg, pos = t.select(dim, 0), t.select(dim, 1)
    return torch.where(pos > neg, pos, -neg)


@HEADS.register_module()
class LSHead(nn.Module):

    def __init__(self, num_classes, in_channels, feat_channels=256, stacked_convs=4, strides=(4, 8, 16, 32, 64),
                 point_feat_channels=256, num_kernel_points=9, gradient_mul=0.1,
                 point_strides=[8, 16, 32, 64, 128], point_base_scale=4, task='bbox', num_vectors=4,
                 conv_module_type='norm', background_label=None, conv_cfg=None, norm_cfg=None,
                 loss_cls=dict(type='FocalLoss', use_sigmoid=True, gamma=2.0, alpha=0.25, loss_weight=1.0),
                 loss_bbox_init=dict(type='CrossIOULoss', loss_weight=1.0),
                 loss_bbox_refine=dict(type='CrossIOULoss', loss_weight=2.0),
                 loss_segm_init=None, loss_segm_refine=None, loss_pose_init=None, loss_pose_refine=None,
                 train_cfg=None, test_cfg=None, **kwargs):
        super().__init__()
        assert task in TASK_BRANCHES, task
        self.task, self.branches = task, TASK_BRANCHES[task]
        self.num_classes = self.cls_out_channels = num_classes
# ... 185 lines not shown
    def forward(self, feats, after_init=None):
        nl = len(feats)
        shapes = [tuple(f.shape[2:]) for f in feats]
        base_offset = self.dcn_base_offset.type_as(feats[0])
        cls_feats = self._run_tower(self.cls_convs, feats)
        st = {}
        for b in self.branches:
            tower = self._run_tower(getattr(self, f'{b}_convs'), feats)
            init_conv, init_out = getattr(self, f'pts_{b}_init_conv'), getattr(self, f'pts_{b}_init_out')
            n_sp = self._out_dims(b)[1]
            raw = init_out(self._cat_px(init_conv.forward_multi(tower, relu=True)))
            sp = self.softplus(raw[:, :n_sp])
            reg = self.get_pred_reg(sp, raw[:, n_sp:] if raw.shape[1] > n_sp else None)
            reg = (1 - self.gradient_mul) * reg.detach() + self.gradient_mul * reg
            st[b] = dict(feat=tower, sp_all=sp, sp=self._split_px(sp, shapes),
                         off=self._split_px(reg - base_offset, shapes))

        if after_init is not None:
            after_init({b: st[b]['sp'] for b in self.branches})

        pairs = []
        mults = []
        for l in range(nl):
            bh, bw = cls_feats[l].shape[2:]
            trio = []
            for s in self._level_list(l, nl):
                sh, sw = cls_feats[s].shape[2] / bh, cls_feats[s].shape[3] / bw
                trio.append((sh, sw))
                pairs.append((l, s, sh, sw))
            mults.append(trio)
        driver = self.branches[-1]
        scaled, scaled_cls = {}, None
        for b in self.branches:
            sets = offset_scale_chain(st[b]['off'], mults, copies=2 if b == driver else 1)
            scaled[b] = [t for trio in sets[0] for t in trio]
            if b == driver:
                scaled_cls = [t for trio in sets[1] for t in trio]
        scales = [(p[2], p[3]) for p in pairs]

        def gather(conv, src_feats, offsets):
            return conv.forward_multi([src_feats[p[1]] for p in pairs], offsets, scales, concat=3)

        cls_raw = gather(self.pts_cls_conv, cls_feats, scaled_cls)
        outs = {}
        def fuse(af, fc, raw, feat):
            a = af[0].forward_multi(raw, relu=True)
            if hasattr(fc, 'forward_multi') and 'residuals' in fc.forward_multi.__code__.co_varnames:
                return fc.forward_multi(feat, residuals=a)
            f = fc.forward_multi(feat)
            return [x + y for x, y in zip(a, f)]

        fused = fuse(self.cls_af_dcn_conv, self.cls_feat_conv, cls_raw, cls_feats)
        outs['cls'] = self._split_px(self.pts_cls_out(self._gn_cat(self.cls_GN, fused)), shapes)
        for b in self.branches:
            raw = gather(getattr(self, f'pts_{b}_refine_conv'), st[b]['feat'], scaled[b])
            af, fc = getattr(self, f'{b}_af_dcn_conv'), getattr(self, f'{b}_feat_conv')
            gn, ro = getattr(self, f'{b}_GN'), getattr(self, f'pts_{b}_refine_out')
            fused = fuse(af, fc, raw, st[b]['feat'])
            refine = self.softplus(ro(self._gn_cat(gn, fused)) + st[b]['sp_all'].detach())
            outs[b] = self._split_px(refine, shapes)

        none = [None] * nl
        res = [outs['cls']]
        for b in ('bbox', 'segm', 'pose'):
            res += [st[b]['sp'], outs[b]] if b in self.branches else [none, none]
        return tuple(res)

    def forward_train(self, x, img_metas, gt_bboxes, gt_extremes=None, gt_keypoints=None, gt_masks=None,
                      gt_labels=None, gt_bboxes_ignore=None, proposal_cfg=None, **kwargs):
        pre, stage2, hook = None, [], None
        if SIDE_STREAM_TARGETS and x[0].is_cuda:
            main = torch.cuda.current_stream(x[0].device)
            side = self._side_stream(x[0].device)
            side.wait_stream(main)
            with torch.cuda.stream(side):
                pre = self.init_stage_targets([tuple(f.shape[-2:]) for f in x], x[0], gt_bboxes, gt_extremes, gt_keypoints,
                                              gt_masks, gt_labels, img_metas)

            def hook(init_preds):
                side.wait_stream(main)
                with torch.cuda.stream(side):
                    stage2.append(self.refine_stage_targets(pre, [p.detach() for p in init_preds[self._box_branch()]]))
        outs = self(x, after_init=hook)
        if pre is not None:
            main.wait_stream(side)
        losses = self.loss(*outs, gt_bboxes, gt_extremes, gt_keypoints, gt_masks, gt_labels, img_metas,
                           gt_bboxes_ignore=gt_bboxes_ignore, init_stage=pre, refine_stage=stage2[0] if stage2 else None)
        if proposal_cfg is None:
            return losses
        return losses, self.get_bboxes(*outs, img_metas, cfg=proposal_cfg)

    def get_points(self, featmap_sizes, img_metas, device):
        key = ('points', tuple(tuple(s) for s in featmap_sizes), tuple(tuple(m['pad_shape'][:2]) for m in img_metas),
               str(device))
        hit = self._consts.get(key)
        if hit is not None:
            return hit
        points = [self.point_generators[i].grid_points(featmap_sizes[i], self.point_strides[i], device)
                  for i in range(len(featmap_sizes))]
        flags, all_valid = [], True
        for meta in img_metas:
            per_level = []
            h, w = meta['pad_shape'][:2]
            for i, (fh, fw) in enumerate(featmap_sizes):
                s = self.point_strides[i]
                vh, vw = min(int(np.ceil(h / s)), fh), min(int(np.ceil(w / s)), fw)
                all_valid = all_valid and vh == fh and vw == fw
                per_level.append(self.point_generators[i].valid_flags((fh, fw), (vh, vw), device))
            flags.append(per_level)
        if len(self._consts) > 64:
            self._consts.clear()
        self._consts[key] = (points, flags, all_valid)
        return points, flags, all_valid

    def _dense_targets(self, gt_inds, gt_labels, gt_bboxes, extra):
        pos = gt_inds > 0
        idx = (gt_inds - 1).clamp(min=0)
        posf = pos.unsqueeze(1)
        fields = [('bboxes_gt', gt_bboxes)] + list(extra.items())
        if assigners.NATIVE_ASSIGN and gt_inds.is_cuda and gt_inds.dtype == torch.long and \
                all(v.is_cuda and v.dtype == torch.float32 and v.dim() == 2 for _, v in fields):
            table = gt_bboxes if len(fields) == 1 else torch.cat([v for _, v in fields], dim=1)
            rows = get_backend(table).dense_targets(gt_inds, table)
            gathered = dict(zip([k for k, _ in fields], torch.split(rows, [v.shape[1] for _, v in fields], dim=1)))
        else:
            gathered = {k: torch.where(posf, v[idx], 0.0) for k, v in fields}
        out = dict(bboxes_gt=gathered['bboxes_gt'],
                   bbox_weights=posf.to(gt_bboxes.dtype).expand(-1, 4),
                   labels=torch.where(pos, gt_labels[idx] if gt_labels is not None else torch.ones_like(idx),
                                      self.background_label),
                   label_weights=torch.ones_like(pos, dtype=gt_bboxes.dtype), num_pos=pos.sum())
        for k in extra:
            out[k] = gathered[k]
        return out

    def _assign_image(self, stage, proposals, flags, all_valid, num_level, gt_bboxes, gt_labels, extra, res=None):
        n_all = proposals.shape[0]
        if gt_bboxes.shape[0] == 0:
            zeros = proposals.new_zeros
            out = dict(bboxes_gt=zeros((n_all, 4)), bbox_weights=zeros((n_all, 4)),
                       labels=proposals.new_full((n_all,), self.background_label, dtype=torch.long),
                       label_weights=proposals.new_ones((n_all,)), num_pos=proposals.new_zeros((), dtype=torch.long))
            for k, v in extra.items():
                out[k] = zeros((n_all, v.shape[1]))
            return out
        inside = None if all_valid else flags
        props = proposals if inside is None else proposals[inside]
        if res is not None:
            assert inside is None
        elif stage == 'init':
            res = self.init_assigner.assign(props, gt_bboxes, extra.get('extremes_gt'), None, gt_labels)
        else:
            if inside is not None:
                num_level = [int(f.sum()) for f in torch.split(inside, num_level)]
            res = self.refine_assigner.assign(props, num_level, gt_bboxes, None, gt_labels)
        out = self._dense_targets(res.gt_inds, gt_labels, gt_bboxes, extra)
        if inside is not None:
            full = {}
            for k, v in out.items():
                if k == 'num_pos':
                    full[k] = v
                    continue
                buf = v.new_zeros((n_all,) + tuple(v.shape[1:]))
                buf[inside] = v
                full[k] = buf
            out = full
# ... 403 lines not shown
```

lsnet_amd/ops/dcn.py:

```python
import math

import torch
import torch.nn as nn
import torch.nn.functional as F
from torch.autograd import Function
from torch.autograd.function import once_differentiable
from torch.nn.modules.utils import _pair, _single

from ..cnn.registry import CONV_LAYERS
from . import grad_sink
from .backend import get_backend
from . import conv as _conv
from .conv import Conv2d


def _conv_out(size, k, stride, pad, dil):
    return (size + 2 * pad - (dil * (k - 1) + 1)) // stride + 1


def _same_int(v, what):
    v = _pair(v)
    if v[0] != v[1]:
        raise NotImplementedError(f'{what} must be the same for height and width, got {v}')
    return int(v[0])


def _backend_backward(ctx, inputs, offsets, masks, weight, gos, need):
    sinks_ok = getattr(ctx.backend, 'dcn_sinks_ok', None)
    c = grad_sink.claim([(weight, need['weight']), (ctx.bias_ref, need['bias'])], optional=(1,),
                        allowed=sinks_ok is not None and sinks_ok(inputs, weight))
    kw = dict(sinks=c.sinks) if c.accumulate else {}
    gxs, goffs, gmsks, gw, gb = ctx.backend.dcn_backward(inputs, offsets, masks, weight, gos, ctx.cfg, need, **kw)
    return (gxs, goffs, gmsks, *c.results((gw, gb)))


class _DCNFunction(Function):

    @staticmethod
    def forward(ctx, weight, bias, cfg, n, *tensors):
        inputs, offsets, masks = tensors[:n], tensors[n:2 * n], tensors[2 * n:3 * n]
        backend = get_backend(inputs[0])
        out_hw = []
        for x, off in zip(inputs, offsets):
            if cfg['pyramid']:
                hw = (_conv_out(off.shape[2], weight.shape[2], cfg['stride'], cfg['pad'], cfg['dil']),
                      _conv_out(off.shape[3], weight.shape[3], cfg['stride'], cfg['pad'], cfg['dil']))
            else:
                hw = (_conv_out(x.shape[2], weight.shape[2], cfg['stride'], cfg['pad'], cfg['dil']),
                      _conv_out(x.shape[3], weight.shape[3], cfg['stride'], cfg['pad'], cfg['dil']))
            if not all(s > 0 for s in hw):
                raise ValueError('convolution input is too small (output would be '
                                 f'{x.shape[0]}x{weight.shape[0]}x{hw[0]}x{hw[1]})')
            if tuple(off.shape[2:]) != hw:
                raise RuntimeError(f'invalid spatial size of offset, expected height: {hw[0]} width: {hw[1]}, '
                                   f'but got height: {off.shape[2]} width: {off.shape[3]}')
            if off.shape[1] != cfg['dg'] * (3 if cfg.get('fused_om') else 2) * weight.shape[2] * weight.shape[3]:
                raise RuntimeError('invalid number of channels of offset')
            out_hw.append(hw)
        ctx.cfg, ctx.n, ctx.backend = cfg, n, backend
        ctx.has_bias = bias is not None
        ctx.bias_ref = bias
        ctx.mask_none = [m is None for m in masks]
        ctx.save_for_backward(weight, *inputs, *offsets, *[m for m in masks if m is not None])
        outs = backend.dcn_forward(list(inputs), list(offsets), list(masks), weight, bias, cfg, out_hw)
        cat = int(cfg.get('concat') or 0)
        if cat > 1 and len(outs) == n:
            outs = [torch.cat(outs[j:j + cat], dim=1) for j in range(0, n, cat)]
        return tuple(outs)

    @staticmethod
    @once_differentiable
    def backward(ctx, *grad_outs):
        n, cfg = ctx.n, ctx.cfg
        saved = ctx.saved_tensors
        weight, inputs, offsets = saved[0], saved[1:1 + n], saved[1 + n:1 + 2 * n]
        rest = list(saved[1 + 2 * n:])
        masks = [None if none else rest.pop(0) for none in ctx.mask_none]
        nig = ctx.needs_input_grad
        need = dict(weight=nig[0], bias=ctx.has_bias and nig[1],
                    input=[nig[4 + i] for i in range(n)],
                    offset=[nig[4 + n + i] for i in range(n)],
                    mask=[nig[4 + 2 * n + i] for i in range(n)])
        gos = []
        cat = int(cfg.get('concat') or 0)
        if cat > 1:
            Co = weight.shape[0]
            for j, g in enumerate(grad_outs):
                x, off = inputs[j * cat], offsets[j * cat]
                if g is None:
                    g = x.new_zeros((x.shape[0], cat * Co, off.shape[2], off.shape[3]))
                if x.is_contiguous(memory_format=torch.channels_last):
                    g = g.contiguous(memory_format=torch.channels_last)
                gos += [g.narrow(1, q * Co, Co) for q in range(cat)]
        for i, g in enumerate(grad_outs if cat <= 1 else ()):
            if g is None:
                x, off = inputs[i], offsets[i]
                g = x.new_zeros((x.shape[0], weight.shape[0], off.shape[2], off.shape[3]))
            gos.append(g)
        gxs, goffs, gmsks, gw, gb = _backend_backward(ctx, list(inputs), list(offsets), masks, weight, gos, need)
        gxs = [g if need['input'][i] else None for i, g in enumerate(gxs)]
        goffs = [g if need['offset'][i] else None for i, g in enumerate(goffs)]
        gmsks = [g if (need['mask'][i] and not ctx.mask_none[i]) else None for i, g in enumerate(gmsks)]
        if gw is not None and gw.stride() != weight.stride():
            gw = gw.contiguous(memory_format=torch.channels_last if weight.is_contiguous(
                memory_format=torch.channels_last) and not weight.is_contiguous() else torch.contiguous_format)
        return (gw, gb, None, None, *gxs, *goffs, *gmsks)


class _DCNPackFn(Function):

    @staticmethod
    def forward(ctx, weight, bias, w_off, b_off, cfg, n, *xs):
        backend = get_backend(xs[0])
        pad, dil = cfg['pad'], cfg['dil']
        w_off = w_off.contiguous(memory_format=torch.channels_last)
        offs = _conv.conv_multi_fwd(xs, w_off, b_off, pad, dil, False)
        out_hw = [tuple(o.shape[2:]) for o in offs]
        outs = backend.dcn_forward(list(xs), offs, [None] * n, weight, bias, cfg, out_hw)
        ctx.cfg, ctx.n, ctx.backend = cfg, n, backend
        ctx.bias_ref, ctx.b_off_ref = bias, b_off
        ctx.save_for_backward(weight, w_off, *xs, *offs)
        return tuple(outs)

    @staticmethod
    @once_differentiable
    def backward(ctx, *grad_outs):
        n, cfg = ctx.n, ctx.cfg
        saved = ctx.saved_tensors
        weight, w_off, xs, offs = saved[0], saved[1], saved[2:2 + n], saved[2 + n:2 + 2 * n]
        nig = ctx.needs_input_grad
        need_x = [nig[6 + i] for i in range(n)]
        need_off = nig[2] or nig[3] or any(need_x)
        need = dict(weight=nig[0], bias=ctx.bias_ref is not None and nig[1], input=[True] * n if any(need_x) else [False] * n,
                    offset=[need_off] * n, mask=[False] * n)
        gos = [g if g is not None else x.new_zeros((x.shape[0], weight.shape[0], o.shape[2], o.shape[3]))
               for g, x, o in zip(grad_outs, xs, offs)]
        gxs, goffs, _, gw, gb = _backend_backward(ctx, list(xs), list(offs), [None] * n, weight, gos, need)
        pad, dil = cfg['pad'], cfg['dil']
        if any(need_x):
            gxs = _conv.conv_multi_dgrad(goffs, w_off, xs, pad, dil, accumulate_into=gxs)
        gwo = gbo = None
        if nig[2] or nig[3]:
            gwo, gbo = _conv.conv_multi_wgrad(xs, goffs, w_off, ctx.b_off_ref, pad, dil, nig[2], nig[3])
        return (gw, gb, gwo, gbo, None, None, *[g if nx else None for g, nx in zip(gxs, need_x)])


class _OffsetChainFn(Function):

    @staticmethod
    def forward(ctx, mults, copies, *offs):
        be = get_backend(offs[0])
        ctx.mults, ctx.be, ctx.device, ctx.copies = mults, be, offs[0].device, copies
        ctx.shapes = [tuple(o.shape) for o in offs]
        res = be.offset_chain(list(offs), mults)
        out = [t for trio in res for t in trio]
        if copies == 2:
            out += [t.view(t.shape) for t in out]
        return tuple(out)

    @staticmethod
    @once_differentiable
    def backward(ctx, *grads):
        n = len(ctx.shapes)
        gs = [list(grads[3 * l:3 * l + 3]) + (list(grads[3 * n + 3 * l:3 * n + 3 * l + 3]) if ctx.copies == 2 else [])
              for l in range(n)]
        return (None, None, *ctx.be.offset_chain_backward(ctx.shapes, ctx.device, ctx.mults, gs))


def offset_scale_chain(offs, mults, copies=1):
    offs = list(offs)
    if offs and all(o.is_cuda for o in offs) and len(offs) <= 8 and all(len(m) == 3 for m in mults) and copies in (1, 2):
        be = get_backend(offs[0])
        if all(be.offset_chain_ok(o) for o in offs):
            n = len(offs)
            flat = _OffsetChainFn.apply(tuple(tuple((float(a), float(b)) for a, b in m) for m in mults), copies, *offs)
            return [[list(flat[c * 3 * n + 3 * l:c * 3 * n + 3 * l + 3]) for l in range(n)] for c in range(copies)]
    res = []
    for off, m in zip(offs, mults):
        cur, trio = off, []
        for sh, sw in m:
            mult = _scale_const(float(sh), float(sw), off.shape[1], off.device, off.dtype)
            cur = cur * mult
            trio.append(cur)
        res.append(trio)
    return [res] * copies


_SCALE_CONSTS = {}


def _scale_const(sh, sw, channels, device, dtype):
    key = (sh, sw, channels, str(device), dtype)
    t = _SCALE_CONSTS.get(key)
    if t is None:
        t = torch.tensor([sh, sw], dtype=dtype).repeat(channels // 2).view(1, -1, 1, 1).to(device)
        _SCALE_CONSTS[key] = t
    return t


def dcn_multi(inputs, offsets, masks, weight, bias=None, stride=1, padding=0, dilation=1, groups=1,
              deformable_groups=1, scales=None, pyramid=False, fused_om=False, concat=0):
# ... 242 lines not shown
```

lsnet_amd/ops/hip_backend.py:

```python
import ctypes

import torch

from .. import _lib
from .._lib import ptr, stream
from .._lib import ptr as _ptr, stream as _stream
from .backend import register_backend

_CL = torch.channels_last
CACHE_DCN_IMAGES = __import__('os').environ.get('LSNET_CACHE_DCN_IMAGES', '1') != '0'


def _f32(t, what):
    if t.dtype != torch.float32:
        raise TypeError(f'{what} must be float32, got {t.dtype}')
    return t


def _is_nhwc(t):
    return t.dim() == 4 and t.is_contiguous(memory_format=_CL)


def _dense(t, nhwc):
    if t.is_contiguous() or t.is_contiguous(memory_format=_CL):
# ... 138 lines not shown
    @staticmethod
    def _shape(w, cfg):
        Co, Cg, kh, kw = w.shape
        return _lib.DcnShape(0, Cg * cfg['groups'], 0, 0, Co, 0, 0, kh, kw, cfg['stride'], cfg['pad'],
                             cfg['dil'], cfg['groups'], cfg['dg'], 1.0, 1.0, 1 if cfg.get('fused_om') else 0)

    @staticmethod
    def _mask_view_ptr(om, cfg, kk):
        return om.data_ptr() + 2 * cfg['dg'] * kk * om.stride(1) * om.element_size()

    def _dcn_levels(self, xs, offs, msks, w, cfg, out_hw):
        levels = (_lib.DcnLevel * len(xs))()
        for L, x, off, msk, (Ho, Wo), scale in zip(levels, xs, offs, msks, out_hw, cfg['scales']):
            L.input, L.offset, L.mask = ptr(x), ptr(off), ptr(msk)
            L.off_st = _strides(off)
            if cfg.get('fused_om'):
                L.mask, L.mask_st = self._mask_view_ptr(off, cfg, w.shape[2] * w.shape[3]), _strides(off)
            elif msk is not None:
                L.mask_st = _strides(msk)
            L.B, L.H, L.W, L.Ho, L.Wo = x.shape[0], x.shape[2], x.shape[3], Ho, Wo
            L.scale_h, L.scale_w = scale
        return levels

    @staticmethod
    def _weight_workspace(shape, levels, w, weight, cfg, nhwc, backward):
        if CACHE_DCN_IMAGES and nhwc and w is weight and cfg['groups'] == 1 and isinstance(weight, torch.nn.Parameter):
            shape.workspace, shape.weights_prepared = w.data_ptr(), 1
            if _lib.load().lsn_dcn_prepared_ok(ctypes.byref(shape), len(levels), levels, 1 if backward else 0):
                from .weight_images import weight_image
                try:
                    img = weight_image(w, 2 if backward else 0, 1, cfg['pad'], cfg['dil'])
                    shape.workspace = img.data_ptr()
                    return img
                except NotImplementedError:
                    pass
            shape.weights_prepared = 0
        ws = torch.empty(2 * w.numel(), device=w.device, dtype=torch.float32)
        shape.workspace = ws.data_ptr()
        return ws

    def dcn_forward(self, inputs, offsets, masks, weight, bias, cfg, out_hw):
        lib = _lib.load()
        nhwc, xs, offs, msks, w = self._prep(inputs, offsets, masks, weight)
        n = len(xs)
        shape = self._shape(w, cfg)
        levels = self._dcn_levels(xs, offs, msks, w, cfg, out_hw)
        outs = []
        g = int(cfg.get('concat') or 0)
        Co = w.shape[0]
        wide = None
        if g > 1:
            assert n % g == 0 and all(out_hw[i] == out_hw[i - i % g] and xs[i].shape[0] == xs[i - i % g].shape[0] for i in range(n))
            if nhwc and (g * Co) % 4 == 0:
                wide = [torch.empty((xs[j].shape[0], g * Co) + tuple(out_hw[j]), device=xs[j].device, dtype=torch.float32,
                                    memory_format=_CL) for j in range(0, n, g)]
        for i in range(n):
            if wide is not None:
                out = wide[i // g].narrow(1, (i % g) * Co, Co)
            else:
                out = torch.empty((xs[i].shape[0], Co) + tuple(out_hw[i]), device=xs[i].device, dtype=torch.float32,
                                  memory_format=_CL if nhwc else torch.contiguous_format)
            outs.append(out)
            levels[i].output = ptr(out)
        b = None if bias is None else _f32(bias.contiguous(), 'bias')
        if _lib.split_math():
            ws = self._weight_workspace(shape, levels, w, weight, cfg, nhwc, False)
        if wide is not None:
            shape.out_pitch = g * Co
            if not lib.lsn_dcn_pitched_ok(ctypes.byref(shape), n, levels, 0):
                shape.out_pitch = 0
                wide = None
                outs = [torch.empty(tuple(o.shape), device=o.device, dtype=torch.float32, memory_format=_CL) for o in outs]
                for i in range(n):
                    levels[i].output = ptr(outs[i])
        _lib.check(lib.lsn_dcn_forward(ctypes.byref(shape), n, levels, ptr(w), ptr(b), 1 if nhwc else 0, stream()))
        if g > 1:
            return wide if wide is not None else [torch.cat(outs[j:j + g], dim=1) for j in range(0, n, g)]
        return outs

    @staticmethod
    def dcn_sinks_ok(inputs, weight):
        return all(_is_nhwc(x) for x in inputs) and weight.is_contiguous(memory_format=_CL)

    def dcn_backward(self, inputs, offsets, masks, weight, grad_outs, cfg, need, sinks=None):
        nhwc, xs, offs, msks, w = self._prep(inputs, offsets, masks, weight)
        n = len(xs)
        pitches = {_pixel_pitch(g) for g in grad_outs} if nhwc else {None}
        if len(pitches) == 1 and None not in pitches and pitches != {w.shape[0]}:
            gos = list(grad_outs)
        else:
            gos = [(g.contiguous(memory_format=_CL) if nhwc else g.contiguous()) for g in grad_outs]
        gxs, goffs, gmsks = [], [], []
        shared = {}
        bufs = []
        for i in range(n):
            gx = gx_ret = None
            if need['input'][i]:
                key = (xs[i].data_ptr(), tuple(xs[i].shape)) if nhwc else i
                if key in shared:
                    gx = shared[key]
                else:
                    gx = gx_ret = shared[key] = torch.empty_like(xs[i])
            want_om = need['offset'][i] or (msks[i] is not None and need['mask'][i])
            goffs.append(torch.empty_like(offs[i]) if want_om else None)
            gmsks.append(torch.empty_like(msks[i]) if (want_om and msks[i] is not None) else None)
            gxs.append(gx_ret)
            bufs.append(gx)
        if sinks is not None:
            assert nhwc and w is weight, 'dcn_backward: sinks for a call that dcn_sinks_ok declines'
            gw, gb = sinks
            acc = 1
        else:
            gw = torch.empty_like(w) if (need['weight'] or need['bias']) else None
            gb = torch.empty(w.shape[0], device=w.device, dtype=torch.float32) if need['bias'] else None
            acc = 0
        self._dcn_backward_call(xs, offs, msks, w, gos, bufs, goffs, gmsks, gw, gb, acc, cfg, nhwc, weight)
        return gxs, goffs, gmsks, gw, gb

    def _dcn_backward_call(self, xs, offs, msks, w, gos, gx_bufs, goffs, gmsks, gw, gb, accumulate, cfg, nhwc, weight=None):
        lib = _lib.load()
        n = len(xs)
        shape = self._shape(w, cfg)
        levels = self._dcn_levels(xs, offs, msks, w, cfg, [g.shape[2:] for g in gos])
        for L, go, gx, goff, gmsk in zip(levels, gos, gx_bufs, goffs, gmsks):
            L.grad_output, L.grad_input, L.grad_offset, L.grad_mask = ptr(go), ptr(gx), ptr(goff), ptr(gmsk)
            if cfg.get('fused_om') and goff is not None:
                L.grad_mask = self._mask_view_ptr(goff, cfg, w.shape[2] * w.shape[3])
        nbytes = int(lib.lsn_dcn_backward_workspace_bytes(ctypes.byref(shape), n, levels))
        if nbytes > 0:
            gws = torch.empty(nbytes, device=w.device, dtype=torch.uint8)
            shape.gather_workspace, shape.gather_workspace_bytes = gws.data_ptr(), nbytes
        if cfg['groups'] == 1 and _lib.split_math():
            ws = self._weight_workspace(shape, levels, w, weight, cfg, nhwc, True)
        shape.accumulate_param_grads = 1 if accumulate else 0
        pitch = _pixel_pitch(gos[0]) if nhwc else None
        if pitch is not None and pitch != w.shape[0]:
            shape.out_pitch = pitch
            if not lib.lsn_dcn_pitched_ok(ctypes.byref(shape), n, levels, 1):
                shape.out_pitch = 0
                gos = [g.contiguous(memory_format=_CL) for g in gos]
                for i in range(n):
                    levels[i].grad_output = ptr(gos[i])
        _lib.check(lib.lsn_dcn_backward(ctypes.byref(shape), n, levels, ptr(w), ptr(gw), ptr(gb),
                                        1 if nhwc else 0, stream()))

    @staticmethod
    def _focal_rows(logits, targets, weight=None, d_losses=None):
        if logits.dim() != 2:
            raise ValueError(f'focal loss: logits must be (N, C), got {tuple(logits.shape)}')
        N, C = logits.shape
        if targets.dtype != torch.int64:
            raise TypeError('targets must be int64')
        if targets.numel() != N or targets.device != logits.device:
            raise ValueError(f'focal loss: {targets.numel()} targets on {targets.device} for {N} rows of logits on {logits.device}')
        if weight is not None and (weight.numel() != N or weight.device != logits.device):
            raise ValueError(f'focal loss: {weight.numel()} weights on {weight.device} for {N} rows of logits on {logits.device}')
        if d_losses is not None and (d_losses.shape != logits.shape or d_losses.device != logits.device):
            raise ValueError(f'focal loss: upstream gradient {tuple(d_losses.shape)} for logits {tuple(logits.shape)}')
        return N, C

    def focal_forward(self, logits, targets, gamma, alpha):
        lib = _lib.load()
        logits = _f32(logits, 'logits').contiguous()
        targets = targets.contiguous()
        if targets.dtype != torch.int64:
            raise TypeError('targets must be int64')
        out = torch.empty_like(logits)
        N, C = self._focal_rows(logits, targets)
        _lib.check(lib.lsn_sigmoid_focal_loss_forward(ptr(logits), ptr(targets), ptr(out), N, C, gamma, alpha,
                                                      stream()))
        return out

    def focal_backward(self, logits, targets, d_losses, gamma, alpha):
        lib = _lib.load()
        logits = logits.contiguous()
        d_losses = d_losses.contiguous()
        out = torch.empty_like(logits)
        N, C = self._focal_rows(logits, targets, d_losses=d_losses)
        _lib.check(lib.lsn_sigmoid_focal_loss_backward(ptr(logits), ptr(targets.contiguous()), ptr(d_losses),
                                                       ptr(out), N, C, gamma, alpha, stream()))
        return out

    def focal_sum(self, logits, targets, weight, gamma, alpha):
        lib = _lib.load()
        logits = _f32(logits, 'logits').contiguous()
        out = torch.empty((), device=logits.device, dtype=torch.float32)
        N, C = self._focal_rows(logits, targets, weight)
        w = None if weight is None else _f32(weight, 'weight').contiguous()
        _lib.check(lib.lsn_sigmoid_focal_loss_sum(ptr(logits), ptr(targets.contiguous()), ptr(w), ptr(out), N,
                                                  C, gamma, alpha, stream()))
        return out

    def focal_backward_weighted(self, logits, targets, weight, scale, gamma, alpha):
        lib = _lib.load()
        logits = logits.contiguous()
        out = torch.empty_like(logits)
        N, C = self._focal_rows(logits, targets, weight)
        w = None if weight is None else weight.contiguous()
        scale = scale.to(torch.float32).contiguous()
        _lib.check(lib.lsn_sigmoid_focal_loss_backward_weighted(
            ptr(logits), ptr(targets.contiguous()), ptr(w), ptr(scale), ptr(out), N, C, gamma, alpha, stream()))
        return out

    @staticmethod
    def _level_starts(num_level):
        starts = [0]
        for n in num_level:
            starts.append(starts[-1] + int(n))
        return (ctypes.c_int * len(starts))(*starts), starts[-1]

    def focal_level_sums(self, logits, targets, weight, B, num_level, gamma, alpha):
        lib = _lib.load()
        assert logits.is_contiguous() and targets.is_contiguous() and (weight is None or weight.is_contiguous())
        _f32(logits, 'logits')
        if targets.dtype != torch.int64:
            raise TypeError('targets must be int64')
        starts, nall = self._level_starts(num_level)
        N, C = logits.shape
        assert N == B * nall and targets.numel() == N
        out = torch.empty(len(num_level), device=logits.device, dtype=torch.float32)
        _lib.check(lib.lsn_sigmoid_focal_loss_level_sums(ptr(logits), ptr(targets), ptr(weight), ptr(out), B, nall, C,
                                                         len(num_level), starts, gamma, alpha, stream()))
        return out

    def focal_backward_levels(self, logits, targets, weight, scales, B, num_level, gamma, alpha):
        lib = _lib.load()
        starts, nall = self._level_starts(num_level)
# ... 492 lines not shown
```

Before: 68.97 img/s.

## Batch DCN anchor-list builds across calls and run them on a side stream

Registers each DCN forward's anchor-list build as a pending job. All pending jobs are then built together in batched radix-sort kernels on a side stream, ahead of the backward pass, so the backward can consume the prepared lists instead of sorting inline. This aims to cut per-call kernel launch overhead and overlap the sort work with other computation. The cost is extra device memory held between forward and backward (capped by an env var), a pinned staging ring, and more complex cross-stream synchronization.

Measured after the change: 69.12 img/s (median of 3 runs). About the same (+0.2%).

```diff
diff --git a/include/lsnet_hip.h b/include/lsnet_hip.h
--- a/include/lsnet_hip.h
+++ b/include/lsnet_hip.h
@@ -19,6 +19,12 @@
 typedef enum { LSN_NCHW = 0, LSN_NHWC = 1 } lsn_layout;
 
 typedef struct { int64_t b, c, h, w; } lsn_strides4;
+
+#define LSN_DCN_MAX_LEVELS 16
+typedef struct {
+    int samples, anchors, digit_bits, passes, n_levels;
+    int prow0[LSN_DCN_MAX_LEVELS], abase[LSN_DCN_MAX_LEVELS], has_grad_input[LSN_DCN_MAX_LEVELS];
+} lsn_dcn_lists_sig;
 
 typedef struct {
     int B, C, H, W;
@@ -33,6 +39,9 @@
     int accumulate_param_grads;
     int out_pitch;
     int weights_prepared;
+    void *lists_prepared;
+    int64_t lists_prepared_bytes;
+    lsn_dcn_lists_sig lists_sig;
 } lsn_dcn_shape;
 
 typedef struct {
@@ -69,6 +78,21 @@
 int lsn_dcn_prepared_ok(const lsn_dcn_shape *shape, int n_levels, const lsn_dcn_level *levels, int backward);
 int lsn_dcn_anchor_lists(const lsn_dcn_shape *shape, int n_levels, const lsn_dcn_level *levels, lsn_layout layout,
                          int *sample_anchor, int *list_start, int *list_sample, int64_t *counts, lsn_stream_t stream);
+
+typedef struct {
+    const lsn_dcn_shape *shape;
+    int n_levels;
+    const lsn_dcn_level *levels;
+    void *lists;
+    int64_t lists_bytes;
+    lsn_dcn_lists_sig sig;
+} lsn_dcn_lists_job;
+int64_t lsn_dcn_lists_bytes(const lsn_dcn_shape *shape, int n_levels, const lsn_dcn_level *levels);
+int lsn_dcn_lists_build(int n_jobs, lsn_dcn_lists_job *jobs, lsn_stream_t stream);
+int lsn_dcn_lists_join(lsn_stream_t stream);
+int lsn_dcn_prepared_lists_ok(const lsn_dcn_shape *shape, int n_levels, const lsn_dcn_level *levels);
+int lsn_dcn_lists_export(const lsn_dcn_lists_sig *sig, const void *lists, int *sample_anchor, int *list_start,
+                         int *list_sample, lsn_stream_t stream);
 
 
 int lsn_deform_conv_forward(const float *input, const float *weight, const float *offset, float *output,
diff --git a/lsnet_amd/_lib.py b/lsnet_amd/_lib.py
--- a/lsnet_amd/_lib.py
+++ b/lsnet_amd/_lib.py
@@ -8,6 +8,12 @@
 class Strides4(ctypes.Structure):
     c_name = 'lsn_strides4'
     _fields_ = [('b', ctypes.c_int64), ('c', ctypes.c_int64), ('h', ctypes.c_int64), ('w', ctypes.c_int64)]
+
+
+class DcnListsSig(ctypes.Structure):
+    c_name = 'lsn_dcn_lists_sig'
+    _fields_ = [(k, ctypes.c_int) for k in ('samples', 'anchors', 'digit_bits', 'passes', 'n_levels')] + \
+               [('prow0', ctypes.c_int * 16), ('abase', ctypes.c_int * 16), ('has_grad_input', ctypes.c_int * 16)]
 
 
 class DcnShape(ctypes.Structure):
@@ -19,7 +25,8 @@
                 ('scale_h', ctypes.c_float), ('scale_w', ctypes.c_float), ('mask_is_logit', ctypes.c_int),
                 ('workspace', ctypes.c_void_p), ('gather_workspace', ctypes.c_void_p),
                 ('gather_workspace_bytes', ctypes.c_int64), ('accumulate_param_grads', ctypes.c_int),
-                ('out_pitch', ctypes.c_int), ('weights_prepared', ctypes.c_int)]
+                ('out_pitch', ctypes.c_int), ('weights_prepared', ctypes.c_int),
+                ('lists_prepared', ctypes.c_void_p), ('lists_prepared_bytes', ctypes.c_int64), ('lists_sig', DcnListsSig)]
 
 
 class DcnLevel(ctypes.Structure):
@@ -32,6 +39,12 @@
                 ('Wo', ctypes.c_int), ('scale_h', ctypes.c_float), ('scale_w', ctypes.c_float)]
 
 
+class DcnListsJob(ctypes.Structure):
+    c_name = 'lsn_dcn_lists_job'
+    _fields_ = [('shape', ctypes.POINTER(DcnShape)), ('n_levels', ctypes.c_int), ('levels', ctypes.POINTER(DcnLevel)),
+                ('lists', ctypes.c_void_p), ('lists_bytes', ctypes.c_int64), ('sig', DcnListsSig)]
+
+
 class OffsetChainLevel(ctypes.Structure):
     c_name = 'lsn_offset_chain_level'
     _fields_ = [('off', ctypes.c_void_p), ('out', ctypes.c_void_p * 3), ('gout', ctypes.c_void_p * 6), ('goff', ctypes.c_void_p),
@@ -127,7 +140,7 @@
                [('B', ctypes.c_int * 16), ('H', ctypes.c_int * 16), ('W', ctypes.c_int * 16), ('ms', ctypes.c_float)]
 
 
-STRUCTS = (Strides4, DcnShape, DcnLevel, OffsetChainLevel, WgradBnJob, SgdTensor, SgdGroup, ConvLevel, ConvWprep, GnLevel, GateJob,
+STRUCTS = (Strides4, DcnListsSig, DcnShape, DcnLevel, DcnListsJob, OffsetChainLevel, WgradBnJob, SgdTensor, SgdGroup, ConvLevel, ConvWprep, GnLevel, GateJob,
            DecodeLevel, DecodeSource, CornerLevel, SemLevel, ProfEntry, ProfLaunch)
 
 
@@ -145,6 +158,11 @@
         'lsn_dcn_pitched_ok': (i, [P(DcnShape), i, P(DcnLevel), i]),
         'lsn_dcn_prepared_ok': (i, [P(DcnShape), i, P(DcnLevel), i]),
         'lsn_dcn_anchor_lists': (i, [P(DcnShape), i, P(DcnLevel), i, p, p, p, p, p]),
+        'lsn_dcn_lists_bytes': (q, [P(DcnShape), i, P(DcnLevel)]),
+        'lsn_dcn_lists_build': (i, [i, P(DcnListsJob), p]),
+        'lsn_dcn_lists_join': (i, [p]),
+        'lsn_dcn_prepared_lists_ok': (i, [P(DcnShape), i, P(DcnLevel)]),
+        'lsn_dcn_lists_export': (i, [P(DcnListsSig), p, p, p, p, p]),
         'lsn_deform_conv_forward': (i, [p] * 4 + [i] * 16 + [p]),
         'lsn_deform_conv_backward_input': (i, [p] * 6 + [i] * 16 + [p]),
         'lsn_deform_conv_backward_parameters': (i, [p] * 4 + [i] * 15 + [f, i, p]),
diff --git a/lsnet_amd/csrc/build.py b/lsnet_amd/csrc/build.py
--- a/lsnet_amd/csrc/build.py
+++ b/lsnet_amd/csrc/build.py
@@ -6,7 +6,7 @@
 HERE = os.path.dirname(os.path.abspath(__file__))
 SO = os.path.join(HERE, 'liblsnet_hip.so')
 SOURCES = ['lib_state.hip', 'dcn.hip', 'misc.hip', 'norm.hip', 'conv.hip', 'gconv.hip', 'image.hip', 'loss.hip', 'assign.hip', 'pool.hip', 'decode.hip', 'cpv.hip']
-HEADERS = ['common.h', 'lib_state.h', 'per_stream.h', 'conv_wgrad_route.h', 'conv_route.h', 'dcn_kernels.h', 'dcn_gather_kernels.h', 'dcn_sort_plan.h', 'dcn_grouped_kernels.h', 'conv_kernels.h', 'conv_wgrad_kernels.h', 'dcn_mm_kernels.h', 'prof.h', 'cross_iou_row.h', 'assign_rows.h', 'pool_rows.h', 'decode_rows.h', 'cpv_rows.h', os.path.join('..', '..', 'include', 'lsnet_hip.h')]
+HEADERS = ['common.h', 'lib_state.h', 'per_stream.h', 'conv_wgrad_route.h', 'conv_route.h', 'dcn_kernels.h', 'dcn_gather_kernels.h', 'dcn_sort_plan.h', 'dcn_lists_plan.h', 'dcn_grouped_kernels.h', 'conv_kernels.h', 'conv_wgrad_kernels.h', 'dcn_mm_kernels.h', 'prof.h', 'cross_iou_row.h', 'assign_rows.h', 'pool_rows.h', 'decode_rows.h', 'cpv_rows.h', os.path.join('..', '..', 'include', 'lsnet_hip.h')]
 FLAGS = ['--offload-arch=gfx950', '-O3', '-std=c++17', '-fPIC', '-shared', '-ffp-contract=fast',
          '-fno-slp-vectorize', '-Wno-unused-result']
 
@@ -14,7 +14,7 @@
 def kernel_signature():
     import hashlib
     h = hashlib.sha256()
-    for f in ('common.h', 'conv_kernels.h', 'conv_wgrad_kernels.h', 'conv_wgrad_route.h', 'conv_route.h', 'conv.hip', 'dcn_kernels.h', 'dcn_gather_kernels.h', 'dcn_sort_plan.h', 'dcn_mm_kernels.h', 'dcn_grouped_kernels.h', 'dcn.hip'):
+    for f in ('common.h', 'conv_kernels.h', 'conv_wgrad_kernels.h', 'conv_wgrad_route.h', 'conv_route.h', 'conv.hip', 'dcn_kernels.h', 'dcn_gather_kernels.h', 'dcn_sort_plan.h', 'dcn_lists_plan.h', 'dcn_mm_kernels.h', 'dcn_grouped_kernels.h', 'dcn.hip'):
         with open(os.path.join(HERE, f), 'rb') as fh:
             h.update(fh.read())
     return h.hexdigest()[:16]
@@ -30,7 +30,7 @@
 OBJ_DIR = os.path.join(HERE, 'build')
 UNIT_HEADERS = {
     'lib_state.hip': ['common.h', 'lib_state.h', 'per_stream.h', 'conv_wgrad_route.h', 'prof.h'],
-    'dcn.hip': ['common.h', 'lib_state.h', 'per_stream.h', 'conv_wgrad_route.h', 'conv_route.h', 'dcn_kernels.h', 'dcn_gather_kernels.h', 'dcn_sort_plan.h', 'dcn_mm_kernels.h', 'dcn_grouped_kernels.h', 'conv_kernels.h', 'prof.h'],
+    'dcn.hip': ['common.h', 'lib_state.h', 'per_stream.h', 'conv_wgrad_route.h', 'conv_route.h', 'dcn_kernels.h', 'dcn_gather_kernels.h', 'dcn_sort_plan.h', 'dcn_lists_plan.h', 'dcn_mm_kernels.h', 'dcn_grouped_kernels.h', 'conv_kernels.h', 'prof.h'],
     'conv.hip': ['common.h', 'lib_state.h', 'per_stream.h', 'conv_wgrad_route.h', 'conv_route.h', 'conv_kernels.h', 'conv_wgrad_kernels.h', 'prof.h'],
     'misc.hip': ['common.h', 'lib_state.h', 'per_stream.h', 'conv_wgrad_route.h', 'prof.h'], 'norm.hip': ['common.h', 'lib_state.h', 'per_stream.h', 'conv_wgrad_route.h', 'prof.h'],
     'gconv.hip': ['common.h', 'prof.h'],
diff --git a/lsnet_amd/csrc/dcn.hip b/lsnet_amd/csrc/dcn.hip
--- a/lsnet_amd/csrc/dcn.hip
+++ b/lsnet_amd/csrc/dcn.hip
@@ -534,6 +534,7 @@
     int wg_steps = 0;
     bool own_gather_ws = false;
     GatherPlan plan;
+    unsigned char *lists = nullptr;
     bool gather() const { return data == GATHER_GROUPED || data == GATHER_MM || data == GATHER_XN; }
 };
 
@@ -651,38 +652,194 @@
     });
 }
 
+static_assert(sizeof(ListOne) <= 4096, "a call's own list job travels in the kernel argument");
+static void list_job_levels(ListJob &J, const DcnArgs &a, int n, int na)
+{
+    J = ListJob{};
+    J.a = a;
+    J.KD = a.kh * a.kw * a.dg;
+    J.n = n, J.na = na, J.nblocks = ds_blocks(n);
+    J.a.gtap_rows = n / J.KD;
+}
+
+template <class Src>
+static int launch_list_kernels(const Src &src, int db, int passes, int blocks, int ablocks, int njobs, hipStream_t st)
+{
+    const dim3 grid(blocks), block(DS_THREADS), kblock(DS_KEY_THREADS);
+    const size_t lds = ds_scatter_lds_bytes(db);
+    hipLaunchKernelGGL(dcn_list_keys_kernel<Src>, grid, kblock, 0, st, src, db);
+    for (int p = 0; p < passes; ++p) {
+        if (p > 0) hipLaunchKernelGGL(dcn_list_hist_kernel<Src>, grid, kblock, 0, st, src, p, db);
+        hipLaunchKernelGGL(dcn_list_scan_kernel<Src>, dim3(1 << db, njobs), block, 0, st, src, db);
+        if (p == 0)
+            hipLaunchKernelGGL((dcn_list_scatter_kernel<Src, true, false>), grid, block, lds, st, src, p, db);
+        else if (p + 1 < passes)
+            hipLaunchKernelGGL((dcn_list_scatter_kernel<Src, false, false>), grid, block, lds, st, src, p, db);
+        else
+            hipLaunchKernelGGL((dcn_list_scatter_kernel<Src, false, true>), grid, block, lds, st, src, p, db);
+    }
+    hipLaunchKernelGGL(dcn_list_starts_kernel<Src>, dim3(ablocks), dim3(LB_ANCHOR_BLOCK), 0, st, src);
+    LSN_HIP(hipGetLastError());
+    return 0;
+}
+
 static int build_lists(DcnArgs &a, const GatherPlan &pl, unsigned char *ws, hipStream_t st)
 {
-    int *hist = reinterpret_cast<int *>(ws + pl.o_hist), *start = reinterpret_cast<int *>(ws + pl.o_start);
-    int *key = reinterpret_cast<int *>(ws + pl.o_key);
-    int2 *pairs[2] = {reinterpret_cast<int2 *>(ws + pl.o_pairs), reinterpret_cast<int2 *>(ws + pl.o_pairs) + pl.nsamples};
-    GEntry *ent = reinterpret_cast<GEntry *>(ws + pl.o_ent);
-    Tap *gtap = reinterpret_cast<Tap *>(ws + pl.o_gtap);
-    const int KD = a.kh * a.kw * a.dg, n = pl.nsamples, na = pl.nanchors;
-    a.gtap_rows = n / KD;
-    const int db = ds_digit_bits(na), passes = ds_passes(na), nblocks = ds_blocks(n);
-    const dim3 grid(nblocks), block(DS_THREADS), kblock(DS_KEY_THREADS);
-    const size_t lds = ds_scatter_lds_bytes(db);
-    hipLaunchKernelGGL(dcn_list_keys_kernel, grid, kblock, 0, st, a, n, na, db, nblocks, key, hist, gtap);
-    a.gtap = gtap;
-    for (int p = 0; p < passes; ++p) {
-        const int2 *in = p > 0 ? pairs[(p - 1) & 1] : nullptr;
-        int2 *out = pairs[p & 1];
-        if (p > 0) hipLaunchKernelGGL(dcn_list_hist_kernel, grid, kblock, 0, st, n, p, db, nblocks, in, hist);
-        hipLaunchKernelGGL(dcn_list_scan_kernel, dim3(1 << db), block, 0, st, hist, db, nblocks);
-        if (p == 0)
-            hipLaunchKernelGGL((dcn_list_scatter_kernel<true, false>), grid, block, lds, st, n, na, p, db, nblocks, hist, key, in, out,
-                               ent, (int *)nullptr, gtap, KD, a.gtap_rows);
-        else if (p + 1 < passes)
-            hipLaunchKernelGGL((dcn_list_scatter_kernel<false, false>), grid, block, lds, st, n, na, p, db, nblocks, hist, key, in, out,
-                               ent, (int *)nullptr, gtap, KD, a.gtap_rows);
-        else
-            hipLaunchKernelGGL((dcn_list_scatter_kernel<false, true>), grid, block, lds, st, n, na, p, db, nblocks, hist, key, in,
-                               (int2 *)nullptr, ent, reinterpret_cast<int *>(out), gtap, KD, a.gtap_rows);
-    }
-    const int *skey = reinterpret_cast<const int *>(pairs[(passes - 1) & 1]);
-    hipLaunchKernelGGL(dcn_list_starts_kernel, dim3(cdiv(na + 1, 256)), dim3(256), 0, st, n, na, skey, start);
-    LSN_HIP(hipGetLastError());
+    const int n = pl.nsamples, na = pl.nanchors, passes = ds_passes(na);
+    ListOne one;
+    ListJob &J = one.j;
+    list_job_levels(J, a, n, na);
+    J.hist = reinterpret_cast<int *>(ws + pl.o_hist), J.start = reinterpret_cast<int *>(ws + pl.o_start);
+    J.key = reinterpret_cast<int *>(ws + pl.o_key);
+    J.pair[0] = reinterpret_cast<int2 *>(ws + pl.o_pairs), J.pair[1] = J.pair[0] + n;
+    J.skey = reinterpret_cast<int *>(J.pair[(passes - 1) & 1]);
+    J.ent = reinterpret_cast<GEntry *>(ws + pl.o_ent);
+    J.gtap = reinterpret_cast<Tap *>(ws + pl.o_gtap);
+    a.gtap_rows = J.a.gtap_rows;
+    a.gtap = J.gtap;
+    return launch_list_kernels(one, ds_digit_bits(na), passes, J.nblocks, cdiv(na + 1, LB_ANCHOR_BLOCK), 1, st);
+}
+
+static void lists_sig_of(const DcnArgs &a, const GatherPlan &pl, lsn_dcn_lists_sig *sig)
+{
+    *sig = lsn_dcn_lists_sig{};
+    sig->samples = pl.nsamples, sig->anchors = pl.nanchors;
+    sig->digit_bits = ds_digit_bits(pl.nanchors), sig->passes = ds_passes(pl.nanchors);
+    sig->n_levels = a.nlv;
+    for (int i = 0; i < a.nlv; ++i)
+        sig->prow0[i] = a.lv[i].prow0, sig->abase[i] = a.lv[i].abase, sig->has_grad_input[i] = a.lv[i].gx != nullptr;
+}
+
+static LbCall lists_call_of(const DcnArgs &a)
+{
+    LbCall c{};
+    c.nlv = a.nlv, c.KD = a.kh * a.kw * a.dg;
+    for (int i = 0; i < a.nlv; ++i) {
+        const Lvl &L = a.lv[i];
+        c.lv[i] = LbLevel{L.B, L.H, L.W, L.P, reinterpret_cast<uintptr_t>(L.gx)};
+    }
+    return c;
+}
+
+constexpr int LISTS_RING = 8;
+struct ListsStage {
+    ListJob *host = nullptr;
+    hipEvent_t copied[LISTS_RING] = {};
+    bool used[LISTS_RING] = {};
+    int next = 0;
+    hipEvent_t built = nullptr;
+    bool any_built = false;
+};
+static PerStream<ListsStage> g_lists;
+static int lists_stage(hipStream_t st, ListsStage **out)
+{
+    return g_lists.get(st, "list builds", out, [&](ListsStage &S) {
+        if (int rc = refuse_capture(st, "the staging ring of the list build would be created")) return rc;
+        const size_t bytes = sizeof(ListJob) * LB_MAX_JOBS * LISTS_RING;
+        LSN_HIP(hipHostMalloc(reinterpret_cast<void **>(&S.host), bytes, hipHostMallocDefault));
+        lib_stat(STAT_MALLOCS, 1);
+        for (int i = 0; i < LISTS_RING; ++i) LSN_HIP(hipEventCreateWithFlags(&S.copied[i], hipEventDisableTiming));
+        LSN_HIP(hipEventCreateWithFlags(&S.built, hipEventDisableTiming));
+        return 0;
+    });
+}
+
+static int lists_build_impl(int n_jobs, lsn_dcn_lists_job *jobs, hipStream_t st_main)
+{
+    LSN_CHECK(n_jobs >= 0 && (n_jobs == 0 || jobs), "lsn_dcn_lists_build: %d jobs, jobs %p", n_jobs, (void *)jobs);
+    if (n_jobs == 0) return 0;
+    if (int rc = refuse_capture(st_main, "lsn_dcn_lists_build")) return rc;
+    std::vector<DcnArgs> args(n_jobs);
+    std::vector<lsn_dcn_lists_sig> sigs(n_jobs);
+    std::vector<unsigned char> done(n_jobs, 0);
+    for (int j = 0; j < n_jobs; ++j) {
+        lsn_dcn_lists_job &jb = jobs[j];
+        jb.sig = lsn_dcn_lists_sig{};
+        LSN_CHECK(jb.shape && jb.levels, "lsn_dcn_lists_build: job %d: shape / levels is NULL", j);
+        if (int rc = check_shape(*jb.shape)) return rc;
+        DcnArgs &a = args[j];
+        if (int rc = fill_levels(a, *jb.shape, jb.n_levels, jb.levels, BWD_BM)) return rc;
+        for (int i = 0; i < jb.n_levels; ++i) a.lv[i].gx = jb.levels[i].grad_input;
+        GatherPlan pl;
+        gather_plan(a, pl, true);
+        LSN_CHECK(pl.ok, "lsn_dcn_lists_build: job %d has no anchor lists (lsn_dcn_lists_bytes is 0)", j);
+        lists_sig_of(a, pl, &sigs[j]);
+        lsn_dcn_lists_sig planned;
+        if (!lb_call_sig(lists_call_of(a), &planned) || !lb_sig_equal(planned, sigs[j]))
+            return fail(LSN_ERR_RUNTIME, "lsn_dcn_lists_build: job %d: the batch planner and the backward's plan disagree", j);
+        const LbBuffer buf = lb_buffer(sigs[j]);
+        LSN_CHECK(jb.lists && (reinterpret_cast<uintptr_t>(jb.lists) & 255) == 0 && jb.lists_bytes >= (int64_t)buf.bytes,
+                  "lsn_dcn_lists_build: job %d: lists %p (256-byte aligned), %lld bytes, needs %zu", j, jb.lists,
+                  (long long)jb.lists_bytes, buf.bytes);
+    }
+    SideStream *side = nullptr;
+    if (int rc = side_stream(st_main, &side)) return rc;
+    ListsStage *stage = nullptr;
+    if (int rc = lists_stage(st_main, &stage)) return rc;
+    LSN_HIP(hipEventRecord(side->fork, st_main));
+    LSN_HIP(hipStreamWaitEvent(side->side, side->fork, 0));
+    hipStream_t st = side->side;
+    LbGroup g;
+    while (lb_next_group(n_jobs, sigs.data(), done.data(), sizeof(ListJob), &g)) {
+        float *scr = nullptr;
+        if (int rc = stream_scratch(g.scratch_bytes / sizeof(float) + 64, &scr, st)) return rc;
+        unsigned char *base = reinterpret_cast<unsigned char *>(scr);
+        const int slot = stage->next;
+        stage->next = (slot + 1) % LISTS_RING;
+        if (stage->used[slot] && hipEventQuery(stage->copied[slot]) != hipSuccess) {
+            LSN_HIP(hipEventSynchronize(stage->copied[slot]));
+            lib_stat(STAT_BLOCKING_SYNCS, 1);
+        }
+        ListJob *host = stage->host + (size_t)slot * LB_MAX_JOBS;
+        ListTable tab{};
+        tab.jobs = reinterpret_cast<const ListJob *>(base + g.o_table), tab.njobs = g.njobs;
+        for (int q = 0; q < g.njobs; ++q) {
+            const LbJobPlan &p = g.jobs[q];
+            const lsn_dcn_lists_sig &sg = sigs[p.job];
+            const LbBuffer buf = lb_buffer(sg);
+            unsigned char *lists = reinterpret_cast<unsigned char *>(jobs[p.job].lists);
+            ListJob &J = host[q];
+            list_job_levels(J, args[p.job], sg.samples, sg.anchors);
+            J.key = reinterpret_cast<int *>(base + p.o_key), J.hist = reinterpret_cast<int *>(base + p.o_hist);
+            J.pair[0] = reinterpret_cast<int2 *>(base + p.o_pairs), J.pair[1] = J.pair[0] + sg.samples;
+            J.gtap = reinterpret_cast<Tap *>(lists + buf.o_gtap), J.start = reinterpret_cast<int *>(lists + buf.o_start);
+            J.ent = reinterpret_cast<GEntry *>(lists + buf.o_ent), J.skey = reinterpret_cast<int *>(lists + buf.o_skey);
+            tab.blk0[q] = p.blk0, tab.ablk0[q] = p.ablk0;
+        }
+        tab.blk0[g.njobs] = g.blocks, tab.ablk0[g.njobs] = g.ablocks;
+        LSN_HIP(hipMemcpyAsync(base + g.o_table, host, sizeof(ListJob) * g.njobs, hipMemcpyHostToDevice, st));
+        LSN_HIP(hipEventRecord(stage->copied[slot], st));
+        stage->used[slot] = true;
+        if (int rc = launch_list_kernels(tab, g.db, g.passes, g.blocks, g.ablocks, g.njobs, st)) return rc;
+    }
+    LSN_HIP(hipEventRecord(stage->built, st));
+    stage->any_built = true;
+    for (int j = 0; j < n_jobs; ++j) jobs[j].sig = sigs[j];
+    return 0;
+}
+
+static int lists_join(hipStream_t st)
+{
+    ListsStage *stage = g_lists.find(st);
+    if (stage && stage->any_built) LSN_HIP(hipStreamWaitEvent(st, stage->built, 0));
+    return 0;
+}
+
+static int prepared_lists_check(const lsn_dcn_shape &s, const DcnArgs &a, const GatherPlan &pl, hipStream_t st, bool queried)
+{
+    lsn_dcn_lists_sig own;
+    lists_sig_of(a, pl, &own);
+    if (!lb_sig_valid(s.lists_sig) || !lb_sig_equal(own, s.lists_sig))
+        return fail(LSN_ERR_INVALID, "deformable backward: lists_prepared were planned for another request (%d samples, %d anchors; "
+                    "this call: %d, %d)", s.lists_sig.samples, s.lists_sig.anchors, own.samples, own.anchors);
+    LSN_CHECK((reinterpret_cast<uintptr_t>(s.lists_prepared) & 255) == 0 && s.lists_prepared_bytes >= (int64_t)lb_buffer(own).bytes,
+              "deformable backward: lists_prepared %p (256-byte aligned) of %lld bytes, needs %zu", s.lists_prepared,
+              (long long)s.lists_prepared_bytes, lb_buffer(own).bytes);
+    if (!queried) {
+        ListsStage *stage = g_lists.find(st);
+        LSN_CHECK(stage && stage->any_built, "deformable backward: lists_prepared, but no lsn_dcn_lists_build on this stream");
+        if (int rc = refuse_capture(st, "joining a list build")) return rc;
+    }
     return 0;
 }
 
@@ -693,17 +850,30 @@
     int *start = reinterpret_cast<int *>(ws + pl.o_start);
     GEntry *ent = reinterpret_cast<GEntry *>(ws + pl.o_ent);
     SideStream *side = nullptr;
-    if (r.data == GATHER_MM)
-        if (int rc = side_stream(st_main, &side)) return rc;
-    hipStream_t st = side ? side->side : st_main;
-    if (side) {
-        LSN_HIP(hipEventRecord(side->fork, st_main));
-        LSN_HIP(hipStreamWaitEvent(side->side, side->fork, 0));
-    }
-    if (int rc = build_lists(a, pl, ws, st)) return rc;
-    if (side) {
-        LSN_HIP(hipEventRecord(side->join, side->side));
-        st = st_main;
+    hipStream_t st = st_main;
+    if (r.lists) {
+        lsn_dcn_lists_sig sig;
+        lists_sig_of(a, pl, &sig);
+        const LbBuffer buf = lb_buffer(sig);
+        start = reinterpret_cast<int *>(r.lists + buf.o_start);
+        ent = reinterpret_cast<GEntry *>(r.lists + buf.o_ent);
+        a.gtap = reinterpret_cast<const Tap *>(r.lists + buf.o_gtap);
+        a.gtap_rows = pl.nsamples / (a.kh * a.kw * a.dg);
+        if (r.data != GATHER_MM)
+            if (int rc = lists_join(st_main)) return rc;
+    } else {
+        if (r.data == GATHER_MM)
+            if (int rc = side_stream(st_main, &side)) return rc;
+        if (side) {
+            st = side->side;
+            LSN_HIP(hipEventRecord(side->fork, st_main));
+            LSN_HIP(hipStreamWaitEvent(side->side, side->fork, 0));
+        }
+        if (int rc = build_lists(a, pl, ws, st)) return rc;
+        if (side) {
+            LSN_HIP(hipEventRecord(side->join, side->side));
+            st = st_main;
+        }
     }
     bool any_off = false;
     for (int i = 0; i < a.nlv; ++i) any_off = any_off || a.lv[i].goff || a.lv[i].gmsk;
@@ -741,7 +911,8 @@
             rows[i] = a.lv[i].P;
         }
         if (int rc = conv_mm_rows(a.nlv, xs, outs, rows, a.Co, a.opitch, a.kh * a.kw * a.C, a.wtp, st)) return rc;
-        LSN_HIP(hipStreamWaitEvent(st_main, side->join, 0));
+        if (side) LSN_HIP(hipStreamWaitEvent(st_main, side->join, 0));
+        else if (int rc = lists_join(st_main)) return rc;
         if (any_off) Hb = reinterpret_cast<float *>(ws + pl.o_H);
         break;
     }
@@ -1088,6 +1259,11 @@
                     "(lsn_dcn_pitched_ok)", a.opitch, a.Co);
     if (s.weights_prepared && r.data != DATA_NONE && !r.prepared)
         return fail(LSN_ERR_UNSUPPORTED, "deformable backward: weights_prepared outside the matrix-pipe kernels (lsn_dcn_prepared_ok)");
+    if (s.lists_prepared && r.gather()) {
+        if (layout != LSN_NHWC) return fail(LSN_ERR_UNSUPPORTED, "deformable backward: lists_prepared with LSN_NCHW");
+        if (int rc = prepared_lists_check(s, a, r.plan, st, false)) return rc;
+        r.lists = reinterpret_cast<unsigned char *>(s.lists_prepared);
+    }
     if (r.data != DATA_NONE) {
         if (r.own_gather_ws && !(gws = ws.get(r.plan.bytes / 4 + 64)))
             return fail(LSN_ERR_RUNTIME, "workspace allocation failed");
@@ -1312,6 +1488,62 @@
     return 0;
 }
 
+static bool lists_query(lsn::DcnArgs &a, lsn::DcnRoute &r, const lsn_dcn_shape *shape, int n_levels, const lsn_dcn_level *levels)
+{
+    using namespace lsn;
+    if (!query_args(a, shape, n_levels, levels, 1)) return false;
+    lsn_dcn_shape s = *shape;
+    s.workspace = &s;
+    r = route_backward(a, s, LSN_NHWC, &s, SIZE_MAX, false);
+    return r.gather();
+}
+
+int64_t lsn_dcn_lists_bytes(const lsn_dcn_shape *shape, int n_levels, const lsn_dcn_level *levels)
+{
+    using namespace lsn;
+    DcnArgs a;
+    DcnRoute r;
+    if (!lists_query(a, r, shape, n_levels, levels)) return 0;
+    lsn_dcn_lists_sig sig;
+    lists_sig_of(a, r.plan, &sig);
+    return (int64_t)lb_buffer(sig).bytes;
+}
+
+int lsn_dcn_lists_build(int n_jobs, lsn_dcn_lists_job *jobs, lsn_stream_t stream)
+{
+    return lsn::lists_build_impl(n_jobs, jobs, reinterpret_cast<hipStream_t>(stream));
+}
+
+int lsn_dcn_lists_join(lsn_stream_t stream) { return lsn::lists_join(reinterpret_cast<hipStream_t>(stream)); }
+
+int lsn_dcn_prepared_lists_ok(const lsn_dcn_shape *shape, int n_levels, const lsn_dcn_level *levels)
+{
+    using namespace lsn;
+    DcnArgs a;
+    if (!query_args(a, shape, n_levels, levels, 1) || !shape->lists_prepared) return 0;
+    DcnRoute r = route_backward(a, *shape, LSN_NHWC, shape->gather_workspace, gather_ws_bytes(*shape), false);
+    return r.gather() && prepared_lists_check(*shape, a, r.plan, nullptr, true) == 0 ? 1 : 0;
+}
+
+int lsn_dcn_lists_export(const lsn_dcn_lists_sig *sig, const void *lists, int *sample_anchor, int *list_start,
+                         int *list_sample, lsn_stream_t stream)
+{
+    using namespace lsn;
+    LSN_CHECK(sig && lists && sample_anchor && list_start && list_sample, "lsn_dcn_lists_export: NULL argument");
+    LSN_CHECK(lb_sig_valid(*sig), "lsn_dcn_lists_export: not a signature lsn_dcn_lists_build wrote");
+    hipStream_t st = reinterpret_cast<hipStream_t>(stream);
+    if (int rc = lists_join(st)) return rc;
+    const LbBuffer buf = lb_buffer(*sig);
+    const unsigned char *w = reinterpret_cast<const unsigned char *>(lists);
+    const int n = sig->samples > sig->anchors + 1 ? sig->samples : sig->anchors + 1;
+    LSN_HIP(hipMemsetAsync(sample_anchor, 0xff, sizeof(int) * (size_t)sig->samples, st));
+    hipLaunchKernelGGL(dcn_list_export_sorted_kernel, dim3(cdiv(n, 256)), dim3(256), 0, st, sig->samples, sig->anchors,
+                       reinterpret_cast<const int *>(w + buf.o_skey), reinterpret_cast<const int *>(w + buf.o_start),
+                       reinterpret_cast<const GEntry *>(w + buf.o_ent), sample_anchor, list_start, list_sample);
+    LSN_HIP(hipGetLastError());
+    return 0;
+}
+
 int lsn_dcn_forward(const lsn_dcn_shape *shape, int n_levels, const lsn_dcn_level *levels, const float *weight,
                     const float *bias, lsn_layout layout, lsn_stream_t stream)
 {
diff --git a/lsnet_amd/csrc/dcn_gather_kernels.h b/lsnet_amd/csrc/dcn_gather_kernels.h
--- a/lsnet_amd/csrc/dcn_gather_kernels.h
+++ b/lsnet_amd/csrc/dcn_gather_kernels.h
@@ -1,4 +1,5 @@
 #pragma once
+#include "dcn_lists_plan.h"
 #include "dcn_sort_plan.h"
 
 namespace lsn {
@@ -98,12 +99,50 @@
 }
 
 
-__global__ __launch_bounds__(DS_KEY_THREADS) void dcn_list_keys_kernel(const DcnArgs a, int nsamples, int nanchors, int db, int nblocks,
-                                                                       int *__restrict__ key, int *__restrict__ hist,
-                                                                       Tap *__restrict__ gtap)
+struct ListJob {
+    DcnArgs a;
+    int n, na, nblocks, KD;
+    int *key, *hist, *start, *skey;
+    int2 *pair[2];
+    GEntry *ent;
+    Tap *gtap;
+};
+struct ListOne {
+    ListJob j;
+    __device__ __forceinline__ const ListJob &job(int) const { return j; }
+    __device__ __forceinline__ const ListJob &job_of_block(int b, int *local) const { return *local = b, j; }
+    __device__ __forceinline__ const ListJob &job_of_anchor_block(int b, int *local) const { return *local = b, j; }
+};
+struct ListTable {
+    const ListJob *jobs;
+    int njobs;
+    int blk0[LB_MAX_JOBS + 1], ablk0[LB_MAX_JOBS + 1];
+    __device__ __forceinline__ const ListJob &job(int i) const { return jobs[i]; }
+    __device__ __forceinline__ const ListJob &job_of_block(int b, int *local) const
+    {
+        int i = 0;
+        while (i + 1 < njobs && b >= blk0[i + 1]) ++i;
+        return *local = b - blk0[i], jobs[i];
+    }
+    __device__ __forceinline__ const ListJob &job_of_anchor_block(int b, int *local) const
+    {
+        int i = 0;
+        while (i + 1 < njobs && b >= ablk0[i + 1]) ++i;
+        return *local = b - ablk0[i], jobs[i];
+    }
+};
+
+template <class Src>
+__global__ __launch_bounds__(DS_KEY_THREADS) void dcn_list_keys_kernel(const Src src, int db)
 {
     constexpr int PER = DS_BLOCK / DS_KEY_THREADS;
     __shared__ int h[DS_MAX_DIGITS];
+    int blk;
+    const ListJob &J = src.job_of_block(blockIdx.x, &blk);
+    const DcnArgs &a = J.a;
+    const int nsamples = J.n, nanchors = J.na, nblocks = J.nblocks;
+    int *__restrict__ key = J.key, *__restrict__ hist = J.hist;
+    Tap *__restrict__ gtap = J.gtap;
     const int ndig = 1 << db;
     for (int d = threadIdx.x; d < ndig; d += DS_KEY_THREADS) h[d] = 0;
     __syncthreads();
@@ -113,7 +152,7 @@
     int prow[PER], kd[PER];
 #pragma unroll
     for (int r = 0; r < PER; ++r) {
-        const int s = blockIdx.x * DS_BLOCK + r * DS_KEY_THREADS + threadIdx.x;
+        const int s = blk * DS_BLOCK + r * DS_KEY_THREADS + threadIdx.x;
         const int sc = s < nsamples ? s : nsamples - 1;
         prow[r] = sc / KD, kd[r] = sc - prow[r] * KD;
         const int dgi = kd[r] / K;
@@ -122,7 +161,7 @@
     }
 #pragma unroll
     for (int r = 0; r < PER; ++r) {
-        const int s = blockIdx.x * DS_BLOCK + r * DS_KEY_THREADS + threadIdx.x;
+        const int s = blk * DS_BLOCK + r * DS_KEY_THREADS + threadIdx.x;
         if (s >= nsamples) continue;
         const Lvl &L = *lv[r];
         const int dgi = kd[r] / K, k = kd[r] - dgi * K;
@@ -144,28 +183,33 @@
         atomicAdd(&h[ds_digit(anchor, 0, db)], 1);
     }
     __syncthreads();
-    for (int d = threadIdx.x; d < ndig; d += DS_KEY_THREADS) hist[ds_hist_at(d, blockIdx.x, nblocks)] = h[d];
-}
-
-__global__ __launch_bounds__(DS_KEY_THREADS) void dcn_list_hist_kernel(int nsamples, int pass, int db, int nblocks,
-                                                                       const int2 *__restrict__ in, int *__restrict__ hist)
+    for (int d = threadIdx.x; d < ndig; d += DS_KEY_THREADS) hist[ds_hist_at(d, blk, nblocks)] = h[d];
+}
+
+template <class Src>
+__global__ __launch_bounds__(DS_KEY_THREADS) void dcn_list_hist_kernel(const Src src, int pass, int db)
 {
     constexpr int PER = DS_BLOCK / DS_KEY_THREADS;
     __shared__ int h[DS_MAX_DIGITS];
+    int blk;
+    const ListJob &J = src.job_of_block(blockIdx.x, &blk);
+    const int nsamples = J.n, nblocks = J.nblocks;
+    const int2 *__restrict__ in = J.pair[(pass - 1) & 1];
+    int *__restrict__ hist = J.hist;
     const int ndig = 1 << db;
     for (int d = threadIdx.x; d < ndig; d += DS_KEY_THREADS) h[d] = 0;
     __syncthreads();
     int kk[PER];
 #pragma unroll
     for (int r = 0; r < PER; ++r) {
-        const int i = blockIdx.x * DS_BLOCK + r * DS_KEY_THREADS + threadIdx.x;
+        const int i = blk * DS_BLOCK + r * DS_KEY_THREADS + threadIdx.x;
         kk[r] = i < nsamples ? in[i].x : 0;
     }
 #pragma unroll
     for (int r = 0; r < PER; ++r)
-        if (blockIdx.x * DS_BLOCK + r * DS_KEY_THREADS + threadIdx.x < nsamples) atomicAdd(&h[ds_digit(kk[r], pass, db)], 1);
-    __syncthreads();
-    for (int d = threadIdx.x; d < ndig; d += DS_KEY_THREADS) hist[ds_hist_at(d, blockIdx.x, nblocks)] = h[d];
+        if (blk * DS_BLOCK + r * DS_KEY_THREADS + threadIdx.x < nsamples) atomicAdd(&h[ds_digit(kk[r], pass, db)], 1);
+    __syncthreads();
+    for (int d = threadIdx.x; d < ndig; d += DS_KEY_THREADS) hist[ds_hist_at(d, blk, nblocks)] = h[d];
 }
 
 __device__ __forceinline__ int block_exclusive_sum(int v, int *wsum, int *total)
@@ -191,9 +235,13 @@
     return before + x - v;
 }
 
-__global__ __launch_bounds__(DS_THREADS) void dcn_list_scan_kernel(int *__restrict__ hist, int db, int nblocks)
+template <class Src>
+__global__ __launch_bounds__(DS_THREADS) void dcn_list_scan_kernel(const Src src, int db)
 {
     __shared__ int wsum[DS_WAVES];
+    const ListJob &J = src.job(blockIdx.y);
+    int *__restrict__ hist = J.hist;
+    const int nblocks = J.nblocks;
     int *row = hist + ds_hist_at(blockIdx.x, 0, nblocks);
     int carry = 0;
     for (int base = 0; base < nblocks; base += DS_THREADS) {
@@ -207,17 +255,22 @@
     if (threadIdx.x == 0) hist[ds_hist_at(1 << db, 0, nblocks) + blockIdx.x] = carry;
 }
 
-template <bool FIRST, bool LAST>
-__global__ __launch_bounds__(DS_THREADS) void dcn_list_scatter_kernel(int nsamples, int nanchors, int pass, int db, int nblocks,
-                                                                      const int *__restrict__ hist, const int *__restrict__ key_in,
-                                                                      const int2 *__restrict__ in, int2 *__restrict__ out,
-                                                                      GEntry *__restrict__ ent, int *__restrict__ skey,
-                                                                      const Tap *__restrict__ gtap, int KD, int gtap_rows)
+template <class Src, bool FIRST, bool LAST>
+__global__ __launch_bounds__(DS_THREADS) void dcn_list_scatter_kernel(const Src src, int pass, int db)
 {
     extern __shared__ int ds_lds[];
     __shared__ int wsum[DS_WAVES];
+    int blk;
+    const ListJob &J = src.job_of_block(blockIdx.x, &blk);
+    const int nsamples = J.n, nanchors = J.na, nblocks = J.nblocks, KD = J.KD, gtap_rows = J.a.gtap_rows;
+    const int *__restrict__ hist = J.hist, *__restrict__ key_in = J.key;
+    const int2 *__restrict__ in = J.pair[(pass - 1) & 1];
+    int2 *__restrict__ out = J.pair[pass & 1];
+    GEntry *__restrict__ ent = J.ent;
+    int *__restrict__ skey = J.skey;
+    const Tap *__restrict__ gtap = J.gtap;
     const int lane = threadIdx.x & 63, wave = threadIdx.x >> 6;
-    const int ndig = 1 << db, blk = blockIdx.x;
+    const int ndig = 1 << db;
     int *const cnt = ds_lds, *const gbase = ds_lds + DS_WAVES * ndig;
     int k[DS_ROWS], v[DS_ROWS], loc[DS_ROWS];
 #pragma unroll
@@ -302,9 +355,15 @@
     }
 }
 
-__global__ void dcn_list_starts_kernel(int nsamples, int nanchors, const int *__restrict__ skey, int *__restrict__ start)
-{
-    const int an = blockIdx.x * blockDim.x + threadIdx.x;
+template <class Src>
+__global__ void dcn_list_starts_kernel(const Src src)
+{
+    int blk;
+    const ListJob &J = src.job_of_anchor_block(blockIdx.x, &blk);
+    const int nsamples = J.n, nanchors = J.na;
+    const int *__restrict__ skey = J.skey;
+    int *__restrict__ start = J.start;
+    const int an = blk * LB_ANCHOR_BLOCK + threadIdx.x;
     if (an > nanchors) return;
     int lo = 0, hi = nsamples;
     while (lo < hi) {
@@ -324,6 +383,20 @@
         const int k = key[i];
         sample_anchor[i] = k == nanchors ? -1 : k;
         list_sample[i] = i < start[nanchors] ? ent[i].s : -1;
+    }
+    if (i <= nanchors) list_start[i] = start[i];
+}
+
+__global__ void dcn_list_export_sorted_kernel(int nsamples, int nanchors, const int *__restrict__ skey, const int *__restrict__ start,
+                                              const GEntry *__restrict__ ent, int *__restrict__ sample_anchor,
+                                              int *__restrict__ list_start, int *__restrict__ list_sample)
+{
+    const int i = blockIdx.x * blockDim.x + threadIdx.x;
+    if (i < nsamples) {
+        const bool on_list = i < start[nanchors];
+        const int s = on_list ? ent[i].s : -1;
+        list_sample[i] = s;
+        if (on_list && (unsigned)s < (unsigned)nsamples) sample_anchor[s] = skey[i];
     }
     if (i <= nanchors) list_start[i] = start[i];
 }
diff --git a/lsnet_amd/csrc/dcn_lists_plan.h b/lsnet_amd/csrc/dcn_lists_plan.h
--- /dev/null
+++ b/lsnet_amd/csrc/dcn_lists_plan.h
@@ -0,0 +1,138 @@
+#pragma once
+#include <stddef.h>
+#include <stdint.h>
+
+#include "../../include/lsnet_hip.h"
+#include "dcn_sort_plan.h"
+
+namespace lsn {
+
+constexpr int LB_MAXLV = 16;
+constexpr int LB_MAX_JOBS = 32;
+constexpr int LB_ANCHOR_BLOCK = 256;
+static_assert(LB_MAXLV == LSN_DCN_MAX_LEVELS, "the public signature holds one entry per level");
+
+struct LbLevel {
+    int B, H, W, P;
+    uintptr_t token;
+};
+struct LbCall {
+    int nlv, KD;
+    LbLevel lv[LB_MAXLV];
+};
+
+static inline size_t lb_align(size_t v) { return (v + 255) & ~(size_t)255; }
+
+static inline bool lb_call_sig(const LbCall &c, lsn_dcn_lists_sig *sig)
+{
+    *sig = lsn_dcn_lists_sig{};
+    if (c.nlv < 1 || c.nlv > LB_MAXLV || c.KD < 1) return false;
+    int64_t prow = 0, anchors = 0;
+    bool any = false;
+    lsn_dcn_lists_sig s{};
+    s.n_levels = c.nlv;
+    for (int i = 0; i < c.nlv; ++i) {
+        const LbLevel &L = c.lv[i];
+        if (L.B < 1 || L.H < 1 || L.W < 1 || L.P < 0) return false;
+        if (prow >= ((int64_t)1 << 30)) return false;
+        s.prow0[i] = (int)prow;
+        prow += L.P;
+        if (!L.token) continue;
+        any = true;
+        int first = -1;
+        for (int j = 0; j < i && first < 0; ++j)
+            if (c.lv[j].token == L.token) first = j;
+        if (first < 0) {
+            if (anchors >= ((int64_t)1 << 30)) return false;
+            s.abase[i] = (int)anchors;
+            anchors += (int64_t)L.B * (L.H + 1) * (L.W + 1);
+        } else {
+            if (c.lv[first].B != L.B || c.lv[first].H != L.H || c.lv[first].W != L.W) return false;
+            s.abase[i] = s.abase[first];
+        }
+        s.has_grad_input[i] = 1;
+    }
+    if (!any || prow * c.KD >= ((int64_t)1 << 30) || prow * c.KD < 1 || anchors >= ((int64_t)1 << 30)) return false;
+    s.samples = (int)(prow * c.KD);
+    s.anchors = (int)anchors;
+    s.digit_bits = ds_digit_bits(s.anchors);
+    s.passes = ds_passes(s.anchors);
+    if (s.digit_bits > DS_MAX_DIGIT_BITS) return false;
+    *sig = s;
+    return true;
+}
+
+static inline bool lb_sig_equal(const lsn_dcn_lists_sig &a, const lsn_dcn_lists_sig &b)
+{
+    if (a.samples != b.samples || a.anchors != b.anchors || a.digit_bits != b.digit_bits || a.passes != b.passes ||
+        a.n_levels != b.n_levels)
+        return false;
+    for (int i = 0; i < a.n_levels && i < LB_MAXLV; ++i)
+        if (a.prow0[i] != b.prow0[i] || a.abase[i] != b.abase[i] || a.has_grad_input[i] != b.has_grad_input[i]) return false;
+    return true;
+}
+
+static inline bool lb_sig_valid(const lsn_dcn_lists_sig &s)
+{
+    return s.samples >= 1 && s.samples < (1 << 30) && s.anchors >= 1 && s.anchors < (1 << 30) && s.n_levels >= 1 &&
+           s.n_levels <= LB_MAXLV && s.digit_bits == ds_digit_bits(s.anchors) && s.passes == ds_passes(s.anchors);
+}
+
+struct LbBuffer {
+    size_t o_gtap, o_start, o_ent, o_skey, bytes;
+};
+constexpr size_t LB_TAP_BYTES = 32, LB_ENTRY_BYTES = 16;
+static inline LbBuffer lb_buffer(const lsn_dcn_lists_sig &s)
+{
+    LbBuffer b;
+    size_t o = 0;
+    b.o_gtap = o, o = lb_align(o + ((size_t)s.samples + 1) * LB_TAP_BYTES);
+    b.o_start = o, o = lb_align(o + ((size_t)s.anchors + 1) * sizeof(int));
+    b.o_ent = o, o = lb_align(o + (size_t)s.samples * LB_ENTRY_BYTES);
+    b.o_skey = o, o = lb_align(o + (size_t)s.samples * sizeof(int));
+    b.bytes = o;
+    return b;
+}
+
+struct LbJobPlan {
+    int job;
+    int nblocks, blk0;
+    int ablocks, ablk0;
+    size_t o_key, o_pairs, o_hist;
+};
+struct LbGroup {
+    int db, passes, njobs;
+    int blocks, ablocks;
+    size_t o_table;
+    size_t scratch_bytes;
+    LbJobPlan jobs[LB_MAX_JOBS];
+};
+
+static inline bool lb_next_group(int n, const lsn_dcn_lists_sig *sig, unsigned char *done, size_t table_bytes, LbGroup *g)
+{
+    int first = -1;
+    for (int j = 0; j < n && first < 0; ++j)
+        if (!done[j]) first = j;
+    if (first < 0) return false;
+    g->db = sig[first].digit_bits, g->passes = sig[first].passes, g->njobs = 0;
+    g->blocks = g->ablocks = 0;
+    g->o_table = 0;
+    size_t o = lb_align((size_t)LB_MAX_JOBS * table_bytes);
+    for (int j = first; j < n && g->njobs < LB_MAX_JOBS; ++j) {
+        if (done[j] || sig[j].digit_bits != g->db || sig[j].passes != g->passes) continue;
+        if ((int64_t)g->blocks + ds_blocks(sig[j].samples) >= ((int64_t)1 << 30)) break;
+        LbJobPlan &p = g->jobs[g->njobs++];
+        p.job = j;
+        p.nblocks = ds_blocks(sig[j].samples), p.blk0 = g->blocks;
+        p.ablocks = (sig[j].anchors + 1 + LB_ANCHOR_BLOCK - 1) / LB_ANCHOR_BLOCK, p.ablk0 = g->ablocks;
+        g->blocks += p.nblocks, g->ablocks += p.ablocks;
+        p.o_key = o, o = lb_align(o + (size_t)sig[j].samples * sizeof(int));
+        p.o_pairs = o, o = lb_align(o + (size_t)sig[j].samples * 2 * 2 * sizeof(int));
+        p.o_hist = o, o = lb_align(o + ds_hist_ints(sig[j].samples, sig[j].anchors) * sizeof(int));
+        done[j] = 1;
+    }
+    g->scratch_bytes = o;
+    return true;
+}
+
+}
diff --git a/lsnet_amd/models/dense_heads/ls_head.py b/lsnet_amd/models/dense_heads/ls_head.py
--- a/lsnet_amd/models/dense_heads/ls_head.py
+++ b/lsnet_amd/models/dense_heads/ls_head.py
@@ -12,6 +12,7 @@
 from ...ops.backend import get_backend
 from ...ops import ModulatedDeformConvPack, PyramidDeformConv
 from ...ops.dcn import offset_scale_chain
+from ...ops import dcn_lists
 from ...ops import cross_iou as fused_ciou
 from ...ops.focal import level_rows_ok, level_sums
 from ...ops.streams import side_stream
@@ -363,6 +364,7 @@
                 with torch.cuda.stream(side):
                     stage2.append(self.refine_stage_targets(pre, [p.detach() for p in init_preds[self._box_branch()]]))
         outs = self(x, after_init=hook)
+        dcn_lists.build_pending()
         if pre is not None:
             main.wait_stream(side)
         losses = self.loss(*outs, gt_bboxes, gt_extremes, gt_keypoints, gt_masks, gt_labels, img_metas,
diff --git a/lsnet_amd/ops/dcn.py b/lsnet_amd/ops/dcn.py
--- a/lsnet_amd/ops/dcn.py
+++ b/lsnet_amd/ops/dcn.py
@@ -30,8 +30,17 @@
     c = grad_sink.claim([(weight, need['weight']), (ctx.bias_ref, need['bias'])], optional=(1,),
                         allowed=sinks_ok is not None and sinks_ok(inputs, weight))
     kw = dict(sinks=c.sinks) if c.accumulate else {}
+    if getattr(ctx, 'lists_entry', None) is not None:
+        kw['lists'] = ctx.lists_entry
     gxs, goffs, gmsks, gw, gb = ctx.backend.dcn_backward(inputs, offsets, masks, weight, gos, ctx.cfg, need, **kw)
     return (gxs, goffs, gmsks, *c.results((gw, gb)))
+
+
+def _register_lists(backend, inputs, offsets, masks, weight, cfg, out_hw, need_input):
+    reg = getattr(backend, 'dcn_lists_register', None)
+    if reg is None or not any(need_input):
+        return None
+    return reg(list(inputs), list(offsets), list(masks), weight, cfg, list(out_hw), need_input)
 
 
 class _DCNFunction(Function):
@@ -63,6 +72,8 @@
         ctx.mask_none = [m is None for m in masks]
         ctx.save_for_backward(weight, *inputs, *offsets, *[m for m in masks if m is not None])
         outs = backend.dcn_forward(list(inputs), list(offsets), list(masks), weight, bias, cfg, out_hw)
+        ctx.lists_entry = _register_lists(backend, inputs, offsets, masks, weight, cfg, out_hw,
+                                          [ctx.needs_input_grad[4 + i] for i in range(n)])
         cat = int(cfg.get('concat') or 0)
         if cat > 1 and len(outs) == n:
             outs = [torch.cat(outs[j:j + cat], dim=1) for j in range(0, n, cat)]
@@ -117,6 +128,8 @@
         offs = _conv.conv_multi_fwd(xs, w_off, b_off, pad, dil, False)
         out_hw = [tuple(o.shape[2:]) for o in offs]
         outs = backend.dcn_forward(list(xs), offs, [None] * n, weight, bias, cfg, out_hw)
+        ctx.lists_entry = _register_lists(backend, xs, offs, [None] * n, weight, cfg, out_hw,
+                                          [any(ctx.needs_input_grad[6:6 + n])] * n)
         ctx.cfg, ctx.n, ctx.backend = cfg, n, backend
         ctx.bias_ref, ctx.b_off_ref = bias, b_off
         ctx.save_for_backward(weight, w_off, *xs, *offs)
diff --git a/lsnet_amd/ops/dcn_lists.py b/lsnet_amd/ops/dcn_lists.py
--- /dev/null
+++ b/lsnet_amd/ops/dcn_lists.py
@@ -0,0 +1,122 @@
+import ctypes
+import os
+import weakref
+
+import torch
+
+from .. import _lib
+
+ENABLED = os.environ.get('LSNET_DCN_BATCH_LISTS', '1') != '0'
+CAP_BYTES = int(os.environ.get('LSNET_DCN_LISTS_CAP_MB', '512')) << 20
+
+_pending = []
+_built = []
+_unjoined = []
+_stats = dict(builds=0, built=0, over_cap=0, taken=0, dropped=0)
+
+
+class Entry:
+    __slots__ = ('shape', 'levels', 'n', 'keep', 'need_input', 'mode', 'nbytes', 'buf', 'sig', 'stream', '__weakref__')
+
+    def __init__(self, shape, levels, keep, need_input, nbytes):
+        self.shape, self.levels, self.n, self.keep = shape, levels, len(levels), keep
+        self.need_input, self.mode, self.nbytes = list(need_input), _lib.get_math_mode(), nbytes
+        self.buf = self.sig = self.stream = None
+
+
+def _capturing():
+    return torch.cuda.is_current_stream_capturing()
+
+
+def register(backend, xs, offs, msks, w, cfg, out_hw, need_input):
+    if not ENABLED or not any(need_input) or not xs[0].is_cuda or _capturing():
+        return None
+    shape = backend._shape(w, cfg)
+    levels = backend._dcn_levels(xs, offs, msks, w, cfg, out_hw)
+    for L, x, need in zip(levels, xs, need_input):
+        L.grad_input = x.data_ptr() if need else None
+    nbytes = int(_lib.load().lsn_dcn_lists_bytes(ctypes.byref(shape), len(levels), levels))
+    if nbytes <= 0:
+        return None
+    ent = Entry(shape, levels, (list(offs), [m for m in msks if m is not None]), need_input, nbytes)
+    _pending.append(weakref.ref(ent))
+    return ent
+
+
+def _alive(refs):
+    return [e for e in (r() for r in refs) if e is not None]
+
+
+def held_bytes():
+    live = [e for e in _alive(_built) if e.buf is not None]
+    _built[:] = [weakref.ref(e) for e in live]
+    return sum(e.nbytes for e in live)
+
+
+def _settle():
+    if _unjoined:
+        _lib.check(_lib.load().lsn_dcn_lists_join(_lib.stream()))
+        del _unjoined[:]
+
+
+def build_pending():
+    live = _alive(_pending)
+    del _pending[:]
+    if not live or not ENABLED or _capturing():
+        return 0
+    _settle()
+    room = CAP_BYTES - held_bytes()
+    todo = []
+    for e in live:
+        if e.nbytes <= room:
+            room -= e.nbytes
+            todo.append(e)
+        else:
+            _stats['over_cap'] += 1
+    if not todo:
+        return 0
+    lib = _lib.load()
+    jobs = (_lib.DcnListsJob * len(todo))()
+    dev = torch.device('cuda', torch.cuda.current_device())
+    for J, e in zip(jobs, todo):
+        e.buf = torch.empty(e.nbytes, device=dev, dtype=torch.uint8)
+        J.shape, J.n_levels, J.levels = ctypes.pointer(e.shape), e.n, e.levels
+        J.lists, J.lists_bytes = e.buf.data_ptr(), e.nbytes
+    st = _lib.stream()
+    try:
+        _lib.check(lib.lsn_dcn_lists_build(len(todo), jobs, st))
+    except Exception:
+        for e in todo:
+            e.buf = None
+        raise
+    for J, e in zip(jobs, todo):
+        e.sig, e.stream, e.keep = _lib.DcnListsSig.from_buffer_copy(J.sig), st, None
+        _built.append(weakref.ref(e))
+        _unjoined.append(e.buf)
+    _stats['builds'] += 1
+    _stats['built'] += len(todo)
+    return len(todo)
+
+
+def take(ent, need_input):
+    if ent is None or not ENABLED or _capturing():
+        return None
+    if ent.buf is None and ent.keep is not None and any(r() is ent for r in _pending):
+        build_pending()
+    if ent.buf is None:
+        return None
+    if list(need_input) != ent.need_input or _lib.get_math_mode() != ent.mode or _lib.stream() != ent.stream:
+        _stats['dropped'] += 1
+        return None
+    return ent.buf, ent.sig
+
+
+def taken(ent):
+    _stats['taken'] += 1
+    del _unjoined[:]
+    ent.buf = None
+
+
+def stats():
+    _pending[:] = [weakref.ref(e) for e in _alive(_pending)]
+    return dict(pending=len(_pending), held_bytes=held_bytes(), unjoined=len(_unjoined), **_stats)
diff --git a/lsnet_amd/ops/hip_backend.py b/lsnet_amd/ops/hip_backend.py
--- a/lsnet_amd/ops/hip_backend.py
+++ b/lsnet_amd/ops/hip_backend.py
@@ -244,7 +244,14 @@
     def dcn_sinks_ok(inputs, weight):
         return all(_is_nhwc(x) for x in inputs) and weight.is_contiguous(memory_format=_CL)
 
-    def dcn_backward(self, inputs, offsets, masks, weight, grad_outs, cfg, need, sinks=None):
+    def dcn_lists_register(self, inputs, offsets, masks, weight, cfg, out_hw, need_input):
+        from . import dcn_lists
+        if not dcn_lists.ENABLED or not any(need_input):
+            return None
+        nhwc, xs, offs, msks, w = self._prep(inputs, offsets, masks, weight)
+        return dcn_lists.register(self, xs, offs, msks, w, cfg, out_hw, need_input) if nhwc else None
+
+    def dcn_backward(self, inputs, offsets, masks, weight, grad_outs, cfg, need, sinks=None, lists=None):
         nhwc, xs, offs, msks, w = self._prep(inputs, offsets, masks, weight)
         n = len(xs)
         pitches = {_pixel_pitch(g) for g in grad_outs} if nhwc else {None}
@@ -276,10 +283,12 @@
             gw = torch.empty_like(w) if (need['weight'] or need['bias']) else None
             gb = torch.empty(w.shape[0], device=w.device, dtype=torch.float32) if need['bias'] else None
             acc = 0
-        self._dcn_backward_call(xs, offs, msks, w, gos, bufs, goffs, gmsks, gw, gb, acc, cfg, nhwc, weight)
+        self._dcn_backward_call(xs, offs, msks, w, gos, bufs, goffs, gmsks, gw, gb, acc, cfg, nhwc, weight,
+                                lists=lists if nhwc else None, need_input=need['input'])
         return gxs, goffs, gmsks, gw, gb
 
-    def _dcn_backward_call(self, xs, offs, msks, w, gos, gx_bufs, goffs, gmsks, gw, gb, accumulate, cfg, nhwc, weight=None):
+    def _dcn_backward_call(self, xs, offs, msks, w, gos, gx_bufs, goffs, gmsks, gw, gb, accumulate, cfg, nhwc, weight=None,
+                           lists=None, need_input=None):
         lib = _lib.load()
         n = len(xs)
         shape = self._shape(w, cfg)
@@ -303,8 +312,18 @@
                 gos = [g.contiguous(memory_format=_CL) for g in gos]
                 for i in range(n):
                     levels[i].grad_output = ptr(gos[i])
+        prepared = None
+        if lists is not None:
+            from . import dcn_lists
+            prepared = dcn_lists.take(lists, need_input)
+            if prepared is not None:
+                shape.lists_prepared, shape.lists_prepared_bytes, shape.lists_sig = prepared[0].data_ptr(), prepared[0].numel(), prepared[1]
+                if not lib.lsn_dcn_prepared_lists_ok(ctypes.byref(shape), n, levels):
+                    shape.lists_prepared, shape.lists_prepared_bytes, prepared = None, 0, None
         _lib.check(lib.lsn_dcn_backward(ctypes.byref(shape), n, levels, ptr(w), ptr(gw), ptr(gb),
                                         1 if nhwc else 0, stream()))
+        if prepared is not None:
+            dcn_lists.taken(lists)
 
     @staticmethod
     def _focal_rows(logits, targets, weight=None, d_losses=None):
```
